# gMedAI-Lab/GAViKO

Hardware: AMD Instinct MI355X
Metric: MRI volumes/sec (fwd+bwd) ViT-B/16 gaviko, 120x160x160 (higher is better)
Workload: dtype bf16

## Files before the change

gaviko_amd/csrc/attention_bwd.hip:

```cpp
#include "attention_common.hpp"
#include "../../include/gaviko_hip.h"

namespace gvk {

template <int QT, bool DROP>
__global__ __launch_bounds__(256, 2) void attn_bwd_dkdv_kernel(const bf16* __restrict__ qkv, const bf16* __restrict__ d_o,
                                                            const float* __restrict__ lse, const float* __restrict__ delta,
                                                            bf16* __restrict__ dqkv, int T, int H, int ld_qkv, int ld_o, float dk_scale,
                                                            AttnDrop dr, int need_rows) {
  constexpr int NSB = QT / 32;
  constexpr int kTileQ = QT * 128;
  constexpr int kBuf = 2 * kTileQ + 2 * 128 * 4;
  extern __shared__ __attribute__((aligned(16))) char smem[];
  int bh, kblk;
  xcd_group_block(blockIdx.x, (T + 127) / 128, gridDim.x / ((T + 127) / 128), bh, kblk);
  const int b = bh / H, head = bh - b * H, k0 = kblk * 128;
  if (k0 >= need_rows) return;
  const int lane = lane_id(), wave = wave_id();
  const int r31 = lane & 31, hh = lane >> 5;
  const int inner = H * 64;
  const bf16* qbase = qkv + (size_t)b * T * ld_qkv + head * 64;
  const bool active = k0 + wave * 32 < T;

  const int key = k0 + wave * 32 + r31;
  const int keyc = min(key, T - 1);
  bf16x8 kf[4], vf[4];
#pragma unroll
  for (int ks = 0; ks < 4; ++ks) {
    kf[ks] = *(const bf16x8*)(qbase + inner + (size_t)keyc * ld_qkv + 16 * ks + 8 * hh);
    vf[ks] = *(const bf16x8*)(qbase + 2 * inner + (size_t)keyc * ld_qkv + 16 * ks + 8 * hh);
  }
  [[maybe_unused]] unsigned int akey = 0u;
  if constexpr (DROP) akey = attn_key(dr.seed + *dr.seed_ptr, b * H + head);

  const int nqt = (T + QT - 1) / QT;
  const int nB = (int)gridDim.x / (((T + 127) / 128) * H);
  const __amdgpu_buffer_rsrc_t rq = __builtin_amdgcn_make_buffer_rsrc((void*)qkv, 0, nB * T * ld_qkv * 2, 0x00020000);
  const __amdgpu_buffer_rsrc_t rd = __builtin_amdgcn_make_buffer_rsrc((void*)d_o, 0, nB * T * ld_o * 2, 0x00020000);
  const __amdgpu_buffer_rsrc_t rl = __builtin_amdgcn_make_buffer_rsrc((void*)(wave < 2 ? lse : delta), 0, nB * H * T * 4, 0x00020000);
  const int rsub = lane >> 3, slot = lane & 7;
  int voq[NSB], vod[NSB];
#pragma unroll
  for (int r = 0; r < NSB; ++r) {
    const int row = r * 32 + wave * 8 + rsub;
    const int col = head * 64 + ((slot ^ attn_swz(row)) << 3);
    voq[r] = ((b * T + row) * ld_qkv + col) * 2;
    vod[r] = ((b * T + row) * ld_o + col) * 2;
  }
  const int lrow = (wave & 1) * 64 + lane;
  const int vol = ((b * H + head) * T + lrow) * 4;
  auto stage = [&](int buf, int qt) {
    char* sQ = smem + buf * kBuf;
    char* sD = sQ + kTileQ;
    char* sL = sD + kTileQ;
    const bool last = qt == nqt - 1;
    const int soq = qt * QT * ld_qkv * 2, sod = qt * QT * ld_o * 2, sol = qt * QT * 4;
#pragma unroll
    for (int r = 0; r < NSB; ++r) {
      const int over = last ? max(qt * QT + r * 32 + wave * 8 + rsub - (T - 1), 0) : 0;
      const int vq = voq[r] - over * ld_qkv * 2, vd = vod[r] - over * ld_o * 2;
      __builtin_amdgcn_raw_ptr_buffer_load_lds(rq, (GVK_LDS void*)(sQ + (r * 32 + wave * 8) * 128), 16, vq, soq, 0, 0);
      __builtin_amdgcn_raw_ptr_buffer_load_lds(rd, (GVK_LDS void*)(sD + (r * 32 + wave * 8) * 128), 16, vd, sod, 0, 0);
    }
    const int overl = last ? max(qt * QT + lrow - (T - 1), 0) : 0;
    const int vl = vol - overl * 4;
    __builtin_amdgcn_raw_ptr_buffer_load_lds(rl, (GVK_LDS void*)(sL + (wave >> 1) * 512 + (wave & 1) * 256), 4, vl, sol, 0, 0);
  };

  f32x16 dkt[2], dvt[2];
#pragma unroll
  for (int i = 0; i < 2; ++i) { dkt[i] = f32x16{}; dvt[i] = f32x16{}; }
  const bf16x8 sel_s = aug_sel_first(true, hh);
  [[maybe_unused]] const bf16x8 sel_d = aug_sel_second(hh);
  const int g = lane >> 4, tq = (lane & 15) >> 2, tp = lane & 3;
  stage(0, 0);
  __syncthreads();
  for (int qt = 0; qt < nqt; ++qt) {
    const int buf = qt & 1;
    if (qt + 1 < nqt) stage(buf ^ 1, qt + 1);
    if (active) {
      const char* sQ0 = smem + buf * kBuf;
      const char* sD0 = sQ0 + kTileQ;
      const float* sL0 = (const float*)(sD0 + kTileQ);
      auto scores = [&](int sub, f32x16& s, f32x16& dp) {
        const int qrow0 = qt * QT + sub * 32;
        const char* sQ = sQ0 + sub * 32 * 128;
        const char* sD = sD0 + sub * 32 * 128;
        const float l2 = sL0[sub * 32 + r31] * 1.44269504088896340736f;
        const float dl = DROP ? 0.f : sL0[128 + sub * 32 + r31];
        const bf16x8 qaug = aug_const(l2, qrow0 + r31 >= T, dl, hh);
        s = __builtin_amdgcn_mfma_f32_32x32x16_bf16(qaug, sel_s, f32x16{}, 0, 0, 0);
        if constexpr (DROP) dp = f32x16{};
        else dp = __builtin_amdgcn_mfma_f32_32x32x16_bf16(qaug, sel_d, f32x16{}, 0, 0, 0);
#pragma unroll
        for (int ks = 0; ks < 4; ++ks) {
          const int chunk = 2 * ks + hh;
          const bf16x8 qa = *(const bf16x8*)(sQ + r31 * 128 + ((chunk ^ attn_swz(r31)) << 4));
          const bf16x8 da = *(const bf16x8*)(sD + r31 * 128 + ((chunk ^ attn_swz(r31)) << 4));
          s = __builtin_amdgcn_mfma_f32_32x32x16_bf16(qa, kf[ks], s, 0, 0, 0);
          dp = __builtin_amdgcn_mfma_f32_32x32x16_bf16(da, vf[ks], dp, 0, 0, 0);
        }
      };
      auto soft = [&](int sub, f32x16& s, f32x16& dp) {
        [[maybe_unused]] const int qrow0 = qt * QT + sub * 32;
#pragma unroll
        for (int r = 0; r < 16; ++r) {
          const float pr = __builtin_amdgcn_exp2f(s[r]);
          if constexpr (DROP) {
            const unsigned int qq = (unsigned int)(qrow0 + (r & 3) + 8 * (r >> 2) + 4 * hh);
            const float mm = attn_drop_scale(akey, qq * (unsigned int)T + (unsigned int)key, dr.thresh, dr.inv_keep);
            const float dlr = sL0[128 + sub * 32 + (r & 3) + 8 * (r >> 2) + 4 * hh];
            s[r] = pr * mm;
            dp[r] = pr * (dp[r] * mm - dlr);
          } else {
            s[r] = pr;
          }
        }
        if constexpr (!DROP) {
#pragma unroll
          for (int r = 0; r < 16; r += 2) {
            typedef float f32x2_ __attribute__((ext_vector_type(2)));
            const f32x2_ pp = {s[r], s[r + 1]}, dd = {dp[r], dp[r + 1]};
            const f32x2_ o = pp * dd;
            dp[r] = o[0]; dp[r + 1] = o[1];
          }
        }
      };
      auto grads = [&](int sub, const f32x16& s, const f32x16& dp) {
        const char* sQ = sQ0 + sub * 32 * 128;
        const char* sD = sD0 + sub * 32 * 128;
#pragma unroll
        for (int sk = 0; sk < 2; ++sk) {
          bf16x8 pf, dsf;
#pragma unroll
          for (int j = 0; j < 8; ++j) { pf[j] = (bf16)s[8 * sk + j]; dsf[j] = (bf16)dp[8 * sk + j]; }
          const int q0r = 16 * sk + 4 * (g >> 1);
#pragma unroll
          for (int db = 0; db < 2; ++db) {
            const int chunk = db * 4 + 2 * (g & 1) + (tp >> 1);
            const int ra = q0r + tq, rb = q0r + 8 + tq;
            const int oa = ra * 128 + ((chunk ^ attn_swz(ra)) << 4) + (tp & 1) * 8;
            const int ob = rb * 128 + ((chunk ^ attn_swz(rb)) << 4) + (tp & 1) * 8;
            const bf16x4 da0 = lds_read_tr16(sD + oa), da1 = lds_read_tr16(sD + ob);
            const bf16x4 qa0 = lds_read_tr16(sQ + oa), qa1 = lds_read_tr16(sQ + ob);
            const bf16x8 dof = {da0[0], da0[1], da0[2], da0[3], da1[0], da1[1], da1[2], da1[3]};
            const bf16x8 qf = {qa0[0], qa0[1], qa0[2], qa0[3], qa1[0], qa1[1], qa1[2], qa1[3]};
            dvt[db] = __builtin_amdgcn_mfma_f32_32x32x16_bf16(dof, pf, dvt[db], 0, 0, 0);
            dkt[db] = __builtin_amdgcn_mfma_f32_32x32x16_bf16(qf, dsf, dkt[db], 0, 0, 0);
          }
        }
      };
      constexpr bool PIPE = !DROP;
      f32x16 sc[PIPE ? 2 : 1], dpc[PIPE ? 2 : 1];
      if constexpr (PIPE) scores(0, sc[0], dpc[0]);
#pragma unroll
      for (int sub = 0; sub < NSB; ++sub) {
        const bool more = sub + 1 < NSB && qt * QT + (sub + 1) * 32 < T;
        constexpr int kCurMask = PIPE ? 1 : 0;
        const int cur = sub & kCurMask;
        if constexpr (PIPE) {
          if (more) scores(sub + 1, sc[(sub + 1) & kCurMask], dpc[(sub + 1) & kCurMask]);
        } else {
          scores(sub, sc[0], dpc[0]);
        }
        if constexpr (PIPE) __builtin_amdgcn_sched_barrier(0);
        soft(sub, sc[cur], dpc[cur]);
        if constexpr (PIPE) __builtin_amdgcn_sched_barrier(0);
        grads(sub, sc[cur], dpc[cur]);
        if constexpr (PIPE) __builtin_amdgcn_sched_barrier(0);
        if (!more) break;
      }
    }
    __syncthreads();
  }
  if (!active) return;
  const int kw = k0 + wave * 32;
  bf16* dk_rows = dqkv + ((size_t)b * T + kw) * ld_qkv + inner + head * 64;
  store_rows_t(dkt, dk_scale, smem + wave * 8192, dk_rows, (size_t)ld_qkv, T - kw, lane);
  store_rows_t(dvt, 1.0f, smem + wave * 8192 + 4096, dk_rows + inner, (size_t)ld_qkv, T - kw, lane);
}

template <int KB, bool DROP>
__global__ __launch_bounds__(256, 2) void attn_bwd_dq_kernel(const bf16* __restrict__ qkv, const bf16* __restrict__ o_fwd, const bf16* __restrict__ d_o,
                                                          const float* __restrict__ lse, float* __restrict__ delta,
                                                          bf16* __restrict__ dqkv, int T, int H, int ld_qkv, int ld_o, float scale,
                                                          AttnDrop dr, int need_rows) {
  constexpr int NKB = KB / 32;
  constexpr int kTileBytes = KB * 128;
  extern __shared__ __attribute__((aligned(16))) char smem[];
  int bh, qblk;
  xcd_group_block(blockIdx.x, (T + 127) / 128, gridDim.x / ((T + 127) / 128), bh, qblk);
  const int b = bh / H, head = bh - b * H, q0 = qblk * 128;
  const int lane = lane_id(), wave = wave_id();
  const int r31 = lane & 31, hh = lane >> 5;
  const int inner = H * 64;
  const bf16* base = qkv + (size_t)b * T * ld_qkv + head * 64;
  const bool active = q0 + wave * 32 < T;
  const int q = q0 + wave * 32 + r31;
  const int qc = min(q, T - 1);
  bf16x8 qf[4], dof[4];
  float del = 0.f;
#pragma unroll
  for (int ks = 0; ks < 4; ++ks) {
    qf[ks] = *(const bf16x8*)(base + (size_t)qc * ld_qkv + 16 * ks + 8 * hh);
    dof[ks] = *(const bf16x8*)(d_o + ((size_t)b * T + qc) * ld_o + head * 64 + 16 * ks + 8 * hh);
    const bf16x8 of = *(const bf16x8*)(o_fwd + ((size_t)b * T + qc) * ld_o + head * 64 + 16 * ks + 8 * hh);
#pragma unroll
    for (int j = 0; j < 8; ++j) del += (float)of[j] * (float)dof[ks][j];
  }
  del = half_sum(del);
  if (hh == 0 && q < T) delta[((size_t)b * H + head) * T + q] = del;
  if (q0 >= need_rows) return;
  [[maybe_unused]] unsigned int akey = 0u, qoff = 0u;
  if constexpr (DROP) {
    akey = attn_key(dr.seed + *dr.seed_ptr, b * H + head);
    qoff = (unsigned int)q * (unsigned int)T;
  }
  const float l2 = lse[((size_t)b * H + head) * T + qc] * 1.44269504088896340736f;
  const bf16x8 qaug = aug_const(l2, true, DROP ? 0.f : del, hh);
  [[maybe_unused]] const bf16x8 sel_d = aug_sel_second(hh);

  const int nkt = (T + KB - 1) / KB;
  const int nB = (int)gridDim.x / (((T + 127) / 128) * H);
  const __amdgpu_buffer_rsrc_t rsrc = __builtin_amdgcn_make_buffer_rsrc((void*)qkv, 0, nB * T * ld_qkv * 2, 0x00020000);
  const int rsub = lane >> 3, slot = lane & 7;
  int vo[NKB], vo_last[NKB];
#pragma unroll
  for (int r = 0; r < NKB; ++r) {
    const int row = r * 32 + wave * 8 + rsub;
    const int col = inner + head * 64 + ((slot ^ attn_swz(row)) << 3);
    vo[r] = ((b * T + row) * ld_qkv + col) * 2;
    vo_last[r] = ((b * T + row - max((nkt - 1) * KB + row - (T - 1), 0)) * ld_qkv + col) * 2;
  }
  auto stage = [&](int buf, int kt) {
    char* sK = smem + buf * 2 * kTileBytes;
    char* sV = sK + kTileBytes;
#pragma unroll
    for (int r = 0; r < NKB; ++r) {
      const int v = (kt == nkt - 1) ? vo_last[r] : vo[r];
      const int so = kt * KB * ld_qkv * 2;
      __builtin_amdgcn_raw_ptr_buffer_load_lds(rsrc, (GVK_LDS void*)(sK + (r * 32 + wave * 8) * 128), 16, v, so, 0, 0);
      __builtin_amdgcn_raw_ptr_buffer_load_lds(rsrc, (GVK_LDS void*)(sV + (r * 32 + wave * 8) * 128), 16, v, so + inner * 2, 0, 0);
    }
  };

  f32x16 dqt[2];
  dqt[0] = f32x16{};
  dqt[1] = f32x16{};
  const int g = lane >> 4, tq = (lane & 15) >> 2, tp = lane & 3;
  stage(0, 0);
  __syncthreads();
  for (int kt = 0; kt < nkt; ++kt) {
    const int buf = kt & 1;
    if (kt + 1 < nkt) stage(buf ^ 1, kt + 1);
    if (active) {
      const char* sK = smem + buf * 2 * kTileBytes;
      const char* sV = sK + kTileBytes;
      auto scores = [&](int kb, f32x16& st, f32x16& dpt) {
        const int row = kb * 32 + r31;
        const bf16x8 sel_s = aug_sel_first(kt * KB + row >= T, hh);
        st = __builtin_amdgcn_mfma_f32_32x32x16_bf16(sel_s, qaug, f32x16{}, 0, 0, 0);
        if constexpr (DROP) dpt = f32x16{};
        else dpt = __builtin_amdgcn_mfma_f32_32x32x16_bf16(sel_d, qaug, f32x16{}, 0, 0, 0);
#pragma unroll
        for (int ks = 0; ks < 4; ++ks) {
          const int chunk = 2 * ks + hh;
          const int off = row * 128 + ((chunk ^ attn_swz(row)) << 4);
          const bf16x8 ka = *(const bf16x8*)(sK + off);
          const bf16x8 va = *(const bf16x8*)(sV + off);
          st = __builtin_amdgcn_mfma_f32_32x32x16_bf16(ka, qf[ks], st, 0, 0, 0);
          dpt = __builtin_amdgcn_mfma_f32_32x32x16_bf16(va, dof[ks], dpt, 0, 0, 0);
        }
      };
      auto soft = [&](int kb, f32x16& st, f32x16& dpt) {
#pragma unroll
        for (int r = 0; r < 16; ++r) {
          float dpv = dpt[r];
          if constexpr (DROP) {
            const int key = kt * KB + kb * 32 + (r & 3) + 8 * (r >> 2) + 4 * hh;
            dpv = dpv * attn_drop_scale(akey, qoff + (unsigned int)key, dr.thresh, dr.inv_keep) - del;
          }
          if constexpr (DROP) st[r] = __builtin_amdgcn_exp2f(st[r]) * dpv;
          else st[r] = __builtin_amdgcn_exp2f(st[r]);
        }
        if constexpr (!DROP) {
#pragma unroll
          for (int r = 0; r < 16; r += 2) {
            typedef float f32x2_ __attribute__((ext_vector_type(2)));
            const f32x2_ pp = {st[r], st[r + 1]}, dd = {dpt[r], dpt[r + 1]};
            const f32x2_ o = pp * dd;
            st[r] = o[0]; st[r + 1] = o[1];
          }
        }
      };
      auto grads = [&](int kb, const f32x16& st) {
#pragma unroll
        for (int s2 = 0; s2 < 2; ++s2) {
          bf16x8 dsf;
#pragma unroll
          for (int j = 0; j < 8; ++j) dsf[j] = (bf16)st[8 * s2 + j];
          const int key0 = kb * 32 + 16 * s2 + 4 * (g >> 1);
#pragma unroll
          for (int db = 0; db < 2; ++db) {
            const int chunk = db * 4 + 2 * (g & 1) + (tp >> 1);
            const int ra = key0 + tq, rb = key0 + 8 + tq;
            const bf16x4 ka0 = lds_read_tr16(sK + ra * 128 + ((chunk ^ attn_swz(ra)) << 4) + (tp & 1) * 8);
            const bf16x4 ka1 = lds_read_tr16(sK + rb * 128 + ((chunk ^ attn_swz(rb)) << 4) + (tp & 1) * 8);
            const bf16x8 kt8 = {ka0[0], ka0[1], ka0[2], ka0[3], ka1[0], ka1[1], ka1[2], ka1[3]};
            dqt[db] = __builtin_amdgcn_mfma_f32_32x32x16_bf16(kt8, dsf, dqt[db], 0, 0, 0);
          }
        }
      };
      f32x16 sc[2], dpc[2];
      scores(0, sc[0], dpc[0]);
#pragma unroll
      for (int kb = 0; kb < NKB; ++kb) {
        if (kb + 1 < NKB) scores(kb + 1, sc[(kb + 1) & 1], dpc[(kb + 1) & 1]);
        __builtin_amdgcn_sched_barrier(0);
        soft(kb, sc[kb & 1], dpc[kb & 1]);
        __builtin_amdgcn_sched_barrier(0);
        grads(kb, sc[kb & 1]);
        __builtin_amdgcn_sched_barrier(0);
      }
    }
    __syncthreads();
  }
  if (!active) return;
  const int qw = q0 + wave * 32;
  store_rows_t(dqt, scale, smem + wave * 4096, dqkv + ((size_t)b * T + qw) * ld_qkv + head * 64, (size_t)ld_qkv, T - qw, lane);
}

__global__ __launch_bounds__(256) void attn_delta_kernel(const bf16* __restrict__ o_fwd, const bf16* __restrict__ d_o, float* __restrict__ delta, int M,
                                                         int T, int H, int ld_o) {
  const int gid = blockIdx.x * 256 + threadIdx.x;
  const int c = gid & 7, rh = gid >> 3;
  const int row = min(rh / H, M - 1), head = rh - (rh / H) * H;
  const size_t off = (size_t)row * ld_o + head * 64 + c * 8;
  const bf16x8 a = *(const bf16x8*)(o_fwd + off), b = *(const bf16x8*)(d_o + off);
  float v = 0.f;
#pragma unroll
  for (int j = 0; j < 8; ++j) v += (float)a[j] * (float)b[j];
  v += __shfl_xor(v, 1, 64);
  v += __shfl_xor(v, 2, 64);
  v += __shfl_xor(v, 4, 64);
  if (c == 0 && rh < M * H) {
    const int bb = row / T, t = row - bb * T;
    delta[((size_t)bb * H + head) * T + t] = v;
  }
}

__device__ __forceinline__ int ds_unit(int keyl, int g, int h) {
  return keyl * 64 + ((g ^ ((keyl >> 2) & 3)) << 4) + ((h ^ ((keyl >> 4) & 1)) << 3);
}

template <int QT, int VAR>
__global__ __launch_bounds__(256, 2) void attn_bwd_fused_kernel(const bf16* __restrict__ qkv, const bf16* __restrict__ d_o, const float* __restrict__ lse,
                                                             const float* __restrict__ delta, bf16* __restrict__ dqkv, float* dq_acc, int* prog,
                                                             int* xcc_tab, int* status, int T, int H, int ld_qkv, int ld_o, float scale, float dk_scale) {
  constexpr int NSB = QT / 32;
  constexpr int kTileQ = QT * 128;
  constexpr int kBuf = 2 * kTileQ + 2 * 128 * 4;
  constexpr int kDS = 128 * 64;
  constexpr int kImg = NSB * kDS;
  static_assert(2 * kImg >= 128 * 128, "the dS^T images first hold the K tile");
  extern __shared__ __attribute__((aligned(16))) char smem[];
  char* const sDSbase = smem + 2 * kBuf;
  int* const stab = (int*)(sDSbase + 2 * kImg);
  const int nkb = (T + 127) / 128, nqt = (T + QT - 1) / QT;
  int bh, kblk;
  xcd_group_block(blockIdx.x, nkb, gridDim.x / nkb, bh, kblk);
  const int b = bh / H, head = bh - b * H, k0 = kblk * 128;
// ... 181 lines not shown
      for (int sb = 0; sb < NSB; ++sb)
#pragma unroll
        for (int qh = 0; qh < 2; ++qh) {
          const int q = qt * QT + sb * 32 + 16 * qh + li;
          const bf16x4 o = {(bf16)(hdq[sb][qh][0] * scale), (bf16)(hdq[sb][qh][1] * scale), (bf16)(hdq[sb][qh][2] * scale), (bf16)(hdq[sb][qh][3] * scale)};
          if (q < T) *(bf16x4*)(dqkv + ((size_t)b * T + q) * ld_qkv + head * 64 + 16 * wave + 4 * G) = o;
        }
    } else if (plain) {
#pragma unroll
      for (int sb = 0; sb < NSB; ++sb)
#pragma unroll
        for (int qh = 0; qh < 2; ++qh) *(f32x4*)((char*)accb + aoff + sb * 8192 + qh * 1024) = hdq[sb][qh];
    } else {
#pragma unroll
      for (int sb = 0; sb < NSB; ++sb)
#pragma unroll
        for (int qh = 0; qh < 2; ++qh)
          __builtin_amdgcn_raw_buffer_store_b128(__builtin_bit_cast(u32x4, hdq[sb][qh]), racc, aoff + sb * 8192 + qh * 1024, 0, 16);
    }
    pend_word = qt;
    pend_val = (last || (VAR & 39) != 0) ? 0 : ppos + 1;
  };

  int qt = start, pos, succ;
  chain(qt, pos, succ);
  if constexpr ((VAR & 1) != 0) pos = 0;
  const int xall = __hip_atomic_load((GVK_GLOBAL int*)(xrow + min(lane, nkb - 1)), __ATOMIC_RELAXED, __HIP_MEMORY_SCOPE_AGENT);
  __builtin_amdgcn_s_waitcnt(0x0F70);
  int xs = succ >= 0 && succ < 64 ? __builtin_amdgcn_readlane(xall, succ & 63) : 0;
  int pv = 0;
  if (nqt > 1) stage(1, start + 1 < nqt ? start + 1 : 0);
  scores(0, 0, start * QT);
  soft();
  int par = 0;
  [[maybe_unused]] unsigned long long ph[6] = {0, 0, 0, 0, 0, 0}, tprev = 0;
#define GVK_PH(k)                                                             \
  if constexpr ((VAR & 64) != 0) {                                            \
    const unsigned long long tnow = __builtin_amdgcn_s_memtime();             \
    if (j >= 2 && j < nqt - 2) ph[k] += tnow - tprev;                         \
    tprev = tnow;                                                             \
  }
  for (int j = 0; j < nqt; ++j) {
    const int buf = j & 1;
    const bool lastm = (VAR & 2) ? true : pos == nkb - 1;
    char* sDS = sDSbase + par * kImg;
    GVK_PH(5)
    grads(buf, 0, sDS);
#pragma unroll
    for (int sb = 1; sb < NSB; ++sb) {
      scores(buf, sb, qt * QT + sb * 32);
      soft();
      grads(buf, sb, sDS + sb * kDS);
    }
    GVK_PH(1)
    if constexpr ((VAR & 128) == 0) asm volatile("s_waitcnt vmcnt(0)" : "+v"(pv) : : "memory");
    GVK_PH(2)
    if constexpr ((VAR & 16) == 0) {
      if (wave == 0 && pos > 0 && pv != pos) {
        for (unsigned spins = 0;; ++spins) {
          __builtin_amdgcn_s_sleep(4);
          pv = __hip_atomic_load((GVK_GLOBAL int*)(progb + qt * 32), __ATOMIC_RELAXED, __HIP_MEMORY_SCOPE_AGENT);
          if (pv == pos) break;
          if (spins > (1u << 16)) { if (lane == 0) atomicAdd(status, 1); break; }
        }
#ifdef GVK_DIAG
        if (lane == 0) atomicAdd(status + 1, 1);
#endif
      }
    }
    if constexpr ((VAR & 128) != 0) {
      __builtin_amdgcn_s_waitcnt(0xC07F);
      __builtin_amdgcn_s_barrier();
    } else {
      __syncthreads();
    }
    GVK_PH(3)
    if (pend_word >= 0 && threadIdx.x == 0)
      __hip_atomic_store((GVK_GLOBAL int*)(progb + pend_word * 32), pend_val, __ATOMIC_RELAXED, __HIP_MEMORY_SCOPE_AGENT);
    pend_word = -1;
    const int h_qt = qt, h_pos = pos;
    const bool h_last = lastm, h_add = pos > 0, h_plain = (VAR & 8) == 0 && xs == my_xcc + 1;
    f32x4 hdq[NSB][2];
    u32x4 hld[NSB][2];
#pragma unroll
    for (int sb = 0; sb < NSB; ++sb)
#pragma unroll
      for (int qh = 0; qh < 2; ++qh) hld[sb][qh] = u32x4{0u, 0u, 0u, 0u};
    if constexpr ((VAR & 37) == 0) {
      const int aoff = qt * NSB * 8192 + wave * 2048 + lane * 16;
#pragma unroll
      for (int sb = 0; sb < NSB; ++sb)
#pragma unroll
        for (int qh = 0; qh < 2; ++qh)
          hld[sb][qh] = __builtin_amdgcn_raw_buffer_load_b128(racc, aoff + sb * 8192 + qh * 1024, 0, 16);
    }
    int qtn = qt + 1 < nqt ? qt + 1 : 0;
    if (j + 1 < nqt) {
      if (j + 2 < nqt) stage(buf, qtn + 1 < nqt ? qtn + 1 : 0);
      chain(qtn, pos, succ);
      if constexpr ((VAR & 1) != 0) pos = 0;
      xs = succ >= 0 && succ < 64 ? __builtin_amdgcn_readlane(xall, succ & 63) : 0;
    } else {
      qtn = qt;
    }
    const int bufn = j + 1 < nqt ? buf ^ 1 : buf;
    if constexpr ((VAR & 16) == 0) {
      if (wave == 0) asm volatile("global_load_dword %0, %1, %2 sc1" : "=v"(pv) : "v"(0), "s"(progb + qtn * 32) : "memory");
    }
    GVK_PH(4)
#pragma unroll
    for (int sb = 0; sb < NSB; ++sb) {
      hdq[sb][0] = f32x4{0.f, 0.f, 0.f, 0.f};
      hdq[sb][1] = f32x4{0.f, 0.f, 0.f, 0.f};
      if constexpr ((VAR & 4) == 0) {
#pragma unroll
        for (int kk = 0; kk < 4; ++kk)
#pragma unroll
          for (int qh = 0; qh < 2; ++qh) {
            const char* im = sDS + sb * kDS + kk * 2048;
            const bf16x4 b0 = lds_read_tr16(im + dsr[qh][0]), b1 = lds_read_tr16(im + dsr[qh][1]);
            const bf16x8 bb = {b0[0], b0[1], b0[2], b0[3], b1[0], b1[1], b1[2], b1[3]};
            hdq[sb][qh] = __builtin_amdgcn_mfma_f32_16x16x32_bf16(ktf[kk], bb, hdq[sb][qh], 0, 0, 0);
          }
      }
    }
    scores(bufn, 0, qtn * QT);
    GVK_PH(0)
    if constexpr ((VAR & 4) == 0 && (VAR & 32) == 0) finish(hdq, hld, h_qt, h_pos, h_add, h_last, h_plain);
    if constexpr ((VAR & 32) != 0) {
      if (hdq[0][0][0] + hdq[NSB - 1][1][3] == 123.456f) atomicAdd(status + 3, 1);
    }
    soft();
    qt = qtn;
    par ^= 1;
  }
#undef GVK_PH
  if constexpr ((VAR & 64) != 0) {
    if (lane == 0 && (blockIdx.x == 3 || blockIdx.x == 100 || blockIdx.x == 259))
      for (int k = 0; k < 6; ++k) ((unsigned long long*)(status + 16))[(blockIdx.x == 3 ? 0 : blockIdx.x == 100 ? 1 : 2) * 32 + wave * 8 + k] = ph[k];
  }
  asm volatile("s_waitcnt vmcnt(0)" ::: "memory");
  __syncthreads();
  if (threadIdx.x == 0) {
    if (pend_word >= 0) __hip_atomic_store((GVK_GLOBAL int*)(progb + pend_word * 32), pend_val, __ATOMIC_RELAXED, __HIP_MEMORY_SCOPE_AGENT);
    __hip_atomic_store((GVK_GLOBAL int*)(xrow + kblk), 0, __ATOMIC_RELAXED, __HIP_MEMORY_SCOPE_AGENT);
  }
  if (!active) return;
  const int kw = k0 + wave * 32;
  bf16* dk_rows = dqkv + ((size_t)b * T + kw) * ld_qkv + inner + head * 64;
  store_rows_t(dkt, dk_scale, smem + wave * 8192, dk_rows, (size_t)ld_qkv, T - kw, lane);
  store_rows_t(dvt, 1.0f, smem + wave * 8192 + 4096, dk_rows + inner, (size_t)ld_qkv, T - kw, lane);
}

template <int KB, bool DROP>
static int launch_attn_bwd(const void* qkv, const void* out, const void* dout, const float* lse, float* delta, void* dqkv, int B, int T, int H,
                           int ld_qkv, int ld_out, float scale, AttnDrop dr, hipStream_t s, int need_rows = 1 << 30) {
  const float dk_scale = 0.69314718055994530942f;
  const dim3 grid(((T + 127) / 128) * H * B);
  constexpr unsigned lds_kv = 2 * (2 * KB * 128 + 2 * 128 * 4), lds_q = 2 * 2 * KB * 128;
  static bool attr = false;
  if (!attr) {
    hipError_t e = hipFuncSetAttribute(reinterpret_cast<const void*>(&attn_bwd_dq_kernel<KB, DROP>), hipFuncAttributeMaxDynamicSharedMemorySize, lds_q);
    if (e == hipSuccess) e = hipFuncSetAttribute(reinterpret_cast<const void*>(&attn_bwd_dkdv_kernel<KB, DROP>), hipFuncAttributeMaxDynamicSharedMemorySize, lds_kv);
    if (e != hipSuccess) return set_error(-3, "hipFuncSetAttribute(attn_bwd): %s", hipGetErrorString(e));
    attr = true;
  }
  GVK_LAUNCH((attn_bwd_dq_kernel<KB, DROP>), grid, dim3(256), lds_q, s, (const bf16*)qkv, (const bf16*)out, (const bf16*)dout, lse, delta, (bf16*)dqkv, T, H,
             ld_qkv, ld_out, scale, dr, need_rows);
  int rc = check_launch("attention_bwd/dq");
  if (rc) return rc;
  GVK_LAUNCH((attn_bwd_dkdv_kernel<KB, DROP>), grid, dim3(256), lds_kv, s, (const bf16*)qkv, (const bf16*)dout, lse, (const float*)delta, (bf16*)dqkv, T, H,
             ld_qkv, ld_out, dk_scale, dr, need_rows);
  return check_launch("attention_bwd/dkdv");
}

}

extern "C" int gvk_attention_bwd_bf16_dropout(const void* qkv, const void* out, const void* dout, const float* lse, float* delta, void* dqkv, int B,
                                              int T, int H, int ld_qkv, int ld_out, float scale, float drop_p, uint64_t seed, const void* seed_ptr,
                                              void* stream) {
  using namespace gvk;
  GVK_REQUIRE(qkv && out && dout && lse && delta && dqkv, "gvk_attention_bwd_bf16: null pointer");
  GVK_REQUIRE(B > 0 && T > 0 && H > 0, "gvk_attention_bwd_bf16: empty shape");
  GVK_REQUIRE(ld_qkv >= 3 * H * 64 && ld_qkv % 8 == 0 && ld_out >= H * 64 && ld_out % 8 == 0,
              "gvk_attention_bwd_bf16: head dim is fixed at 64; ld_qkv=%d ld_out=%d inconsistent with H=%d", ld_qkv, ld_out, H);
  GVK_REQUIRE(drop_p >= 0.f && drop_p < 1.f && (drop_p == 0.f || seed_ptr != nullptr), "gvk_attention_bwd_bf16: drop_p in [0,1) and a seed word");
  GVK_REQUIRE(drop_p == 0.f || (int64_t)T * T < (int64_t)1 << 32, "gvk_attention_bwd_bf16: the dropout mask index (query*T + key) is 32-bit");
  GVK_REQUIRE((int64_t)B * T * ld_qkv * 2 < (int64_t)1 << 31, "gvk_attention_bwd_bf16: the qkv tensor must stay below 2 GiB (32-bit buffer offsets)");
  const AttnDrop dr{seed, (const unsigned long long*)seed_ptr, drop_threshold_u32(drop_p), drop_p > 0.f ? 1.f / (1.f - drop_p) : 1.f};
  hipStream_t s = (hipStream_t)stream;
  int kb = ((T + 95) / 96 * 96 < (T + 127) / 128 * 128) ? 96 : 128;
  if (getenv("GAVIKO_HIP_ATTN_KB") && (atoi(getenv("GAVIKO_HIP_ATTN_KB")) == 96 || atoi(getenv("GAVIKO_HIP_ATTN_KB")) == 128)) kb = atoi(getenv("GAVIKO_HIP_ATTN_KB"));
  if (drop_p > 0.f)
    return launch_attn_bwd<96, true>(qkv, out, dout, lse, delta, dqkv, B, T, H, ld_qkv, ld_out, scale, dr, s);
  return kb == 96 ? launch_attn_bwd<96, false>(qkv, out, dout, lse, delta, dqkv, B, T, H, ld_qkv, ld_out, scale, dr, s)
                  : launch_attn_bwd<128, false>(qkv, out, dout, lse, delta, dqkv, B, T, H, ld_qkv, ld_out, scale, dr, s);
}

static constexpr int kFusedQT = 64;
static size_t fused_slabs(int B, int T, int H) { return (size_t)B * H * ((T + kFusedQT - 1) / kFusedQT) * (kFusedQT / 32); }
static size_t fused_ws_cap(size_t ws_bytes) { return ws_bytes < 1024 ? 0 : (ws_bytes - 1024) / (8192 + 128 + 4); }
static size_t fused_status_off(size_t ws_bytes) { return (fused_ws_cap(ws_bytes) * 132 + 255) / 256 * 256; }

extern "C" size_t gvk_attention_bwd_ws_bytes(int B, int T, int H) {
  if (B <= 0 || T <= 0 || H <= 0) return 0;
  return fused_slabs(B, T, H) * (8192 + 128 + 4) + 1024;
}
extern "C" size_t gvk_attention_bwd_status_offset(size_t ws_bytes) { return fused_status_off(ws_bytes); }

extern "C" int gvk_attention_bwd_bf16_fused(const void* qkv, const void* out, const void* dout, const float* lse, float* delta, void* dqkv, void* ws,
                                            size_t ws_bytes, int B, int T, int H, int ld_qkv, int ld_out, float scale, void* stream) {
  using namespace gvk;
  GVK_REQUIRE(qkv && out && dout && lse && delta && dqkv && ws, "gvk_attention_bwd_bf16_fused: null pointer");
  GVK_REQUIRE(B > 0 && T > 0 && H > 0, "gvk_attention_bwd_bf16_fused: empty shape");
  GVK_REQUIRE(ld_qkv >= 3 * H * 64 && ld_qkv % 8 == 0 && ld_out >= H * 64 && ld_out % 8 == 0,
              "gvk_attention_bwd_bf16_fused: head dim is fixed at 64; ld_qkv=%d ld_out=%d inconsistent with H=%d", ld_qkv, ld_out, H);
  GVK_REQUIRE((int64_t)B * T * ld_qkv * 2 < (int64_t)1 << 31, "gvk_attention_bwd_bf16_fused: the qkv tensor must stay below 2 GiB (32-bit buffer offsets)");
  const size_t need = gvk_attention_bwd_ws_bytes(B, T, H);
  GVK_REQUIRE(ws_bytes >= need && ((uintptr_t)ws & 255) == 0, "gvk_attention_bwd_bf16_fused: workspace of %zu bytes (256-byte aligned) needed, %zu given", need, ws_bytes);
  GVK_REQUIRE(fused_ws_cap(ws_bytes) >= fused_slabs(B, T, H), "gvk_attention_bwd_bf16_fused: workspace layout cannot hold %zu slabs", fused_slabs(B, T, H));
  const size_t off_status = fused_status_off(ws_bytes), off_acc = off_status + 256;
  const size_t nsub = (size_t)((T + kFusedQT - 1) / kFusedQT) * (kFusedQT / 32);
  GVK_REQUIRE(nsub * 8192 < ((size_t)1 << 31) && (T + 127) / 128 <= 256, "gvk_attention_bwd_bf16_fused: sequence too long (32-bit slab offsets, 256 key blocks)");
  hipStream_t s = (hipStream_t)stream;
  constexpr unsigned lds = 2 * (2 * kFusedQT * 128 + 2 * 128 * 4) + 2 * (kFusedQT / 32) * 128 * 64 + 1024;
  static bool attr = false;
  if (!attr) {
    hipError_t e = hipFuncSetAttribute(reinterpret_cast<const void*>(&attn_bwd_fused_kernel<kFusedQT, 0>), hipFuncAttributeMaxDynamicSharedMemorySize, lds);
#ifdef GVK_DIAG
    auto set1 = [&](const void* f) { if (e == hipSuccess) e = hipFuncSetAttribute(f, hipFuncAttributeMaxDynamicSharedMemorySize, lds); };
    set1(reinterpret_cast<const void*>(&attn_bwd_fused_kernel<kFusedQT, 1>)); set1(reinterpret_cast<const void*>(&attn_bwd_fused_kernel<kFusedQT, 3>));
    set1(reinterpret_cast<const void*>(&attn_bwd_fused_kernel<kFusedQT, 7>)); set1(reinterpret_cast<const void*>(&attn_bwd_fused_kernel<kFusedQT, 8>));
    set1(reinterpret_cast<const void*>(&attn_bwd_fused_kernel<kFusedQT, 11>)); set1(reinterpret_cast<const void*>(&attn_bwd_fused_kernel<kFusedQT, 15>));
    set1(reinterpret_cast<const void*>(&attn_bwd_fused_kernel<kFusedQT, 16>)); set1(reinterpret_cast<const void*>(&attn_bwd_fused_kernel<kFusedQT, 64>)); set1(reinterpret_cast<const void*>(&attn_bwd_fused_kernel<kFusedQT, 33>)); set1(reinterpret_cast<const void*>(&attn_bwd_fused_kernel<kFusedQT, 129>)); set1(reinterpret_cast<const void*>(&attn_bwd_fused_kernel<kFusedQT, 144>));
#endif
    if (e != hipSuccess) return set_error(-3, "hipFuncSetAttribute(attn_bwd_fused): %s", hipGetErrorString(e));
    attr = true;
  }
  const int M = B * T;
  GVK_LAUNCH(attn_delta_kernel, dim3((unsigned)(((size_t)M * H * 8 + 255) / 256)), dim3(256), 0, s, (const bf16*)out, (const bf16*)dout, delta, M, T, H, ld_out);
  int rc = check_launch("attention_bwd/delta");
  if (rc) return rc;
  const float dk_scale = 0.69314718055994530942f;
  char* w = (char*)ws;
  const dim3 grid(((T + 127) / 128) * H * B);
#define GVK_FUSED(V)                                                                                                                          \
  GVK_LAUNCH((attn_bwd_fused_kernel<kFusedQT, V>), grid, dim3(256), lds, s, (const bf16*)qkv, (const bf16*)dout, lse, (const float*)delta, \
             (bf16*)dqkv, (float*)(w + off_acc), (int*)w, (int*)w + fused_ws_cap(ws_bytes) * 32, (int*)(w + off_status), T, H, ld_qkv, ld_out, scale, dk_scale)
#ifdef GVK_DIAG
  const int var = diag_env("GAVIKO_HIP_ATTN_VAR") ? atoi(diag_env("GAVIKO_HIP_ATTN_VAR")) : 0;
  if (var == 1) GVK_FUSED(1); else if (var == 3) GVK_FUSED(3); else if (var == 7) GVK_FUSED(7); else if (var == 8) GVK_FUSED(8);
  else if (var == 11) GVK_FUSED(11); else if (var == 15) GVK_FUSED(15); else if (var == 16) GVK_FUSED(16); else if (var == 64) GVK_FUSED(64); else if (var == 33) GVK_FUSED(33); else if (var == 129) GVK_FUSED(129); else if (var == 144) GVK_FUSED(144); else
#endif
  GVK_FUSED(0);
#undef GVK_FUSED
  return check_launch("attention_bwd/fused");
}

extern "C" int gvk_attention_bwd_bf16_rows(const void* qkv, const void* out, const void* dout, const float* lse, float* delta, void* dqkv, int B,
                                           int T, int H, int ld_qkv, int ld_out, float scale, int need_rows, void* stream) {
  using namespace gvk;
  GVK_REQUIRE(qkv && out && dout && lse && delta && dqkv, "gvk_attention_bwd_bf16_rows: null pointer");
  GVK_REQUIRE(B > 0 && T > 0 && H > 0 && need_rows > 0, "gvk_attention_bwd_bf16_rows: empty shape");
  GVK_REQUIRE(ld_qkv >= 3 * H * 64 && ld_qkv % 8 == 0 && ld_out >= H * 64 && ld_out % 8 == 0,
              "gvk_attention_bwd_bf16_rows: head dim is fixed at 64; ld_qkv=%d ld_out=%d inconsistent with H=%d", ld_qkv, ld_out, H);
  GVK_REQUIRE((int64_t)B * T * ld_qkv * 2 < (int64_t)1 << 31, "gvk_attention_bwd_bf16_rows: the qkv tensor must stay below 2 GiB (32-bit buffer offsets)");
  const AttnDrop dr{0, nullptr, 0u, 1.f};
  const int kb = ((T + 95) / 96 * 96 < (T + 127) / 128 * 128) ? 96 : 128;
  return kb == 96 ? launch_attn_bwd<96, false>(qkv, out, dout, lse, delta, dqkv, B, T, H, ld_qkv, ld_out, scale, dr, (hipStream_t)stream, need_rows)
                  : launch_attn_bwd<128, false>(qkv, out, dout, lse, delta, dqkv, B, T, H, ld_qkv, ld_out, scale, dr, (hipStream_t)stream, need_rows);
}

extern "C" int gvk_attention_bwd_bf16(const void* qkv, const void* out, const void* dout, const float* lse, float* delta, void* dqkv, int B,
                                      int T, int H, int ld_qkv, int ld_out, float scale, void* stream) {
  return gvk_attention_bwd_bf16_dropout(qkv, out, dout, lse, delta, dqkv, B, T, H, ld_qkv, ld_out, scale, 0.f, 0, nullptr, stream);
}
```

gaviko_amd/engine.py:

```python
from __future__ import annotations

import os
from typing import Dict, List, Optional

import torch

from . import lib as L
from . import ops
from .engine_common import (GRAPH_WARMUP, PLAN_TIMING, SEED_EMB, SEED_LAYER, SEED_PROMPT, USE_GRAPHS, _ABLATE, _EPI_NAMES, _SIDE_STREAMS, Names,
                            _on)
from .engine_common import evp_highpass_operator
from .engine_gaviko import GavikoPaths
from .engine_peft import PeftPaths

GEMM_MARKS = None


_BB_KINDS = ("vit", "adaptformer", "gaviko", "dvpt", "evp", "vpt", "ssf")


class Engine(GavikoPaths, PeftPaths):
    def __init__(self, kind: str, cfg: dict, params: Dict[str, torch.nn.Parameter], depth, heads, dim, mlp_dim):
        self.kind, self.cfg, self.p = kind, cfg, params
        self.depth, self.heads, self.C, self.mlp = depth, heads, dim, mlp_dim
# ... 161 lines not shown
        if stale:
            conv = self._d(names[0]).reshape(self.C, self.Kp).contiguous()
            w["conv"] = ops.to_operand(conv, None if self.fp32 else w.get("conv"), self.adt)
        if not stale and (not need_dgrad or self._have_dgrad):
            return
        for i in range(self.depth):
            for tag, nm in (("qkv", self.names.qkv_weight(i)), ("out", self.names.attn(i) + ".to_out.0.weight"),
                            ("fc1", self.names.mlp(i) + ".net.1.weight"), ("fc2", self.names.mlp(i) + ".net.4.weight")):
                src = self._d(nm).contiguous()
                if stale and tag == "fc2" and self._fuse_up:
                    buf = w.get(f"fc2{i}")
                    if buf is None:
                        buf = w[f"fc2{i}"] = torch.zeros((self.C, self.ldx), dtype=self.adt, device=src.device)
                    buf[:, :self.mlp].copy_(src)
                elif stale:
                    w[f"{tag}{i}"] = ops.to_operand(src, None if self.fp32 else w.get(f"{tag}{i}"), self.adt)
                if need_dgrad and (stale or not self._have_dgrad):
                    w[f"{tag}{i}_t"] = ops.transpose_operand(src, w.get(f"{tag}{i}_t"), self.adt)
        self._have_dgrad = self._have_dgrad and not stale or need_dgrad
        self._w16_version = version

    def _fold_deps(self) -> List[str]:
        n = []
        for i in range(1, self.depth):
            a = self.names.attn(i)
            n += [self.names.qkv_weight(i), a + ".norm.weight", a + ".norm.bias"]
        return n

    def _ensure_fold(self) -> bool:
        if not self._fold_ln1:
            return False
        names = self._fold_deps()
        version = tuple(self.p[n]._version for n in names) + tuple(self.p[n].data_ptr() for n in names)
        if version == self._fold_version and self._fold:
            return True
        for i in range(1, self.depth):
            a = self.names.attn(i)
            Wq, g, b = self._d(self.names.qkv_weight(i)), self._d(a + ".norm.weight"), self._d(a + ".norm.bias")
            w16 = ops.to_operand((Wq * g[None, :]).contiguous(), self._fold.get(f"w{i}"), self.adt)
            self._fold[f"w{i}"] = w16
            for key, val in ((f"c1_{i}", w16.float().sum(1)),
                             (f"c2_{i}", (Wq * b[None, :]).sum(1))):
                if key in self._fold:
                    self._fold[key].copy_(val)
                else:
                    self._fold[key] = val.contiguous()
        self._fold_version = version
        return True

    def _seed_base(self, train: bool) -> int:
        rank = 0
        try:
            import torch.distributed as dist
            if dist.is_available() and dist.is_initialized():
                rank = dist.get_rank()
        except Exception:
            rank = 0
        x = (torch.initial_seed() & 0xFFFFFFFFFFFF) * 0x9E3779B97F4A7C15 + (rank + 1) * 0xBF58476D1CE4E5B9 + (0x94D049BB133111EB if train else 0)
        x &= (1 << 64) - 1
        x ^= x >> 31
        return 0x5EED0000 ^ (x & 0x3FFFFFFFFFFF0000)

    def invalidate_weights(self, names=None) -> None:
        if names is None or any(n in self._shadowed for n in names):
            self._w16_version = None
        if names is None or any(n in self._fold_names for n in names):
            self._fold_version = None

    def workspace(self, B: int, device, train: bool, keep_attn: bool = False, tag: Optional[str] = None):
        key = (B, train, str(device)) + (("attn",) if keep_attn else ()) + ((tag,) if tag else ())
        if key in self._wss:
            self._ws = self._wss[key]
            return self._ws
        C, T, N, M = self.C, self.T, self.N, B * self.T
        z = lambda r, c, dt: ops.act_zeros(r, c, dt, device)
        f32, bf16 = torch.float32, self.adt
        nsave = self.depth if (train or keep_attn) else 1
        ws = {"key": key, "B": B, "M": M}
        ws["img"] = torch.zeros((B, 1) + tuple(g * p for g, p in zip(self.grid, self.patch)), device=device)
        ws["logits"] = torch.zeros((B, self.K), device=device)
        ws["dlogits"] = torch.zeros((B, self.K), device=device)
        ws["seed"] = torch.full((1,), self._seed_base(train), dtype=torch.int64, device=device)
        ws["cols"] = z(B * N, self.Kp, bf16)
        ws["G"] = [z(M, C, f32) for _ in range(self.depth + 1)] if train else [z(M, C, f32), z(M, C, f32)]
        ws["G1"] = [z(M, C, f32) for _ in range(nsave)]
        ws["xn"] = z(M, C, bf16)
        ws["qkv"] = [z(M, 3 * C, bf16) for _ in range(nsave)]
        ws["ctx"] = [z(M, C, bf16) for _ in range(nsave)]
        ws["lse"] = [torch.zeros((B, self.heads, T), device=device) for _ in range(nsave)]
        ws["pre"] = [z(M, self.ldx, bf16) for _ in range(nsave)] if train else [None]
        ws["act"] = z(M, self.ldx, bf16)
        if self._fuse_up:
            ws["act"][:, self.mlp + 3 * self.Lat: self.mlp + 3 * self.Lat + 2] = 1.0
        ws["stat"] = [[torch.zeros(M, device=device) for _ in range(4)] for _ in range(nsave)]
        ws["pooled"] = torch.zeros((B, C), device=device)
        if self._fold_ln1:
            ws["xg16"] = z(M, C, bf16)
            ws["spart"] = torch.zeros((C // 64) * M * 2, device=device)
        if self.kind == "gaviko":
            Lt, P, BN = self.Lat, self.P, B * N
            ws["Lc"] = [torch.zeros((BN, C), device=device) for _ in range((self.depth + 1) if train else 2)]
            mk = lambda *s: torch.zeros(s, device=device)
            ws["mw"] = [dict(mean=mk(BN), rstd=mk(BN), lat=mk(BN, Lt), qkv=mk(BN, 3 * Lt), ctx=mk(BN, Lt), lse=mk(BN)) for _ in range(nsave)]
            ws["gp"] = [dict(zx=mk(M, Lt), xl=mk(M, Lt), zl=mk(BN, Lt), ll=mk(BN, Lt), imp=mk(B, P), gw=mk(B), enh=mk(B, P, Lt),
                             prm=mk(B, P, Lt), qg=mk(B, P, Lt), ql=mk(B, P, Lt), cg=mk(B, P, Lt), cl=mk(B, P, Lt), lse_g=mk(B, P),
                             lse_l=mk(B, P)) for _ in range(nsave)]
        if self.kind == "evp":
            mk = lambda *s_: torch.zeros(s_, device=device)
            BN, Lp = B * N, self.Lp
            ws["xc"] = z(BN, C, f32)
            ws["hp"] = torch.zeros_like(ws["img"])
            ws["hcols"] = z(BN, self.Kp, f32)
            ws["hc"] = z(BN, 64, f32)
            ws["ev"] = dict(e=mk(BN, Lp), s=mk(BN, Lp), pre=[mk(BN, Lp) for _ in range(nsave)], u=[mk(BN, Lp) for _ in range(nsave)],
                            tmp=z(BN, C, f32))
            if train:
                ws["evb"] = dict(du=mk(BN, Lp), dpre=mk(BN, Lp), ds_tmp=mk(BN, Lp), ds=mk(BN, Lp))
                ws["scratch"] = mk(max(ops.outer_scratch_elems(Lp, self.Kp), 128 * C))
                ws["rscratch"] = mk(32 * (Lp * Lp + Lp + 64))
        if self.kind == "dvpt":
            mk = lambda *s_: torch.zeros(s_, device=device)
            ws["dv"] = [dict(z=mk(M, self.Lat), enh=mk(B, self.P, self.Lat), lse=mk(B, self.P)) for _ in range(nsave)]
        if self.kind == "adaptformer":
            ws["xa"] = z(M, C, bf16)
            ws["ad"] = [dict(mean=torch.zeros(M, device=device), rstd=torch.zeros(M, device=device), h16=z(M, self.adim, bf16))
                        for _ in range(nsave)]
            if train:
                ws["dh16"] = z(M, self.adim, bf16)
                ws["h32"] = torch.zeros((M, self.adim), device=device)
                ws["dh32"] = torch.zeros((M, self.adim), device=device)
        if self.kind == "melo":
            ws["merge32"] = torch.zeros((3 * C, C), device=device)
            if train:
                mk = lambda *s_: torch.zeros(s_, device=device)
                ws["dq32"], ws["dv32"] = mk(M, C), mk(M, C)
                ws["lu"] = dict(uq=mk(M, self.r), uv=mk(M, self.r), duq=mk(M, self.r), duv=mk(M, self.r))
        if self.kind == "vpt":
            R = (self.depth if self.deep else 1) * self.P
            ws["vproj"] = torch.zeros((R, C), device=device)
            ws["Go"] = z(M, C, f32)
            if train:
                ws["dvproj"] = torch.zeros((R, C), device=device)
                ws["dGv"] = z(M, C, f32)
        if train:
            ws["dG"] = [z(M, C, f32), z(M, C, f32)]
            ws["dG16"] = z(M, C, bf16)
            ws["dpre"] = z(M, self.mlp, bf16)
            ws["dx32"] = z(M, C, f32)
            if self._dy16:
                ws["dx16b"] = z(M, C, bf16)
            ws["dctx"] = z(M, C, bf16)
            ws["dqkv"] = z(M, 3 * C, bf16)
            ws["delta"] = torch.zeros((B, self.heads, T), device=device)
            if self.kind == "gaviko":
                Lt, P, BN = self.Lat, self.P, B * N
                mk = lambda *s: torch.zeros(s, device=device)
                ng = ops.gpa_gate_param_count(Lt, P)
                ws["dL"] = [mk(BN, C), mk(BN, C)]
                ws["dGb"] = ops.act_zeros(M, C, torch.float32, device)
                ws["bw"] = dict(dcomb=mk(M, Lt), dimp=mk(B, P), dgw_part=mk(B, P), dqg=mk(B, P, Lt), dql=mk(B, P, Lt), dcg=mk(B, P, Lt),
                                dcl=mk(B, P, Lt), delta_g=mk(B, P), delta_l=mk(B, P), dprm=mk(B, P, Lt), dcls=mk(B, Lt),
                                gate_partials=mk(B, ng), dzx=mk(M, Lt), dzl=[mk(BN, Lt), mk(BN, Lt)],
                                dctx=mk(BN, Lt), dqkv=mk(BN, 3 * Lt), wdelta=mk(BN), dlat=mk(BN, Lt), Q=mk(Lt, C), S=mk(Lt))
                ws["scratch"] = mk(max(ops.outer_scratch_elems(Lt, C), 128 * C, 64 * 3 * Lt * Lt, 64 * ng))
                ws["rscratch"] = mk(32 * (ng + 2 * Lt * Lt + 3 * Lt + 3 * Lt * Lt + 64))
                ws["scratch_l"] = mk(max(ops.outer_scratch_elems(Lt, C), 128 * C))
                ws["rscratch_l"] = mk(32 * (3 * Lt * Lt + Lt + 64))
                if self._pgrad:
                    nct = (C + 63) // 64
                    ws["pscratch"] = mk(ops.param_grads_scratch_elems(Lt, [nct, nct], [ng, Lt * Lt, Lt, Lt * Lt, Lt, Lt]))
                    ws["pscratch_l"] = mk(ops.param_grads_scratch_elems(Lt, [nct, nct, (3 * Lt + 63) // 64], []))
                    ws["ptick"] = torch.zeros(ops.PGRAD_TICKETS, dtype=torch.int32, device=device)
                    ws["ptick_l"] = torch.zeros(ops.PGRAD_TICKETS, dtype=torch.int32, device=device)
            elif self.kind == "dvpt":
                Lt, P = self.Lat, self.P
                mk = lambda *s_: torch.zeros(s_, device=device)
                ws["dvb"] = dict(dcomb=mk(M, Lt), dz=mk(M, Lt), delta=mk(B, P))
                ws["scratch"] = mk(max(ops.outer_scratch_elems(Lt, C), 128 * C))
                ws["rscratch"] = mk(32 * (Lt + 64))
            elif self.kind == "evp":
                pass
            else:
                if self.kind == "ssf":
                    ws["ssf_scratch"] = torch.zeros(64 * 2 * max(self.mlp, 3 * C), device=device)
                    ws["ssf_tmp"] = torch.zeros(2 * C, device=device)
                    ws["ssf_stat"] = [torch.zeros(M, device=device), torch.zeros(M, device=device)]
                lat = {"adaptformer": 64, "melo": getattr(self, "r", 4)}.get(self.kind, 1)
                ws["scratch"] = torch.zeros(max(128 * C, ops.outer_scratch_elems(lat, C)), device=device)
        self._ws = self._wss[key] = ws
        return ws

    def _stream(self, name):
        st = self._streams.get(name)
        if st is None:
            key = (torch.cuda.current_device(), name)
            st = _SIDE_STREAMS.get(key)
            if st is not None:
                self._streams[name] = st
                return st
            st = self._streams[name] = _SIDE_STREAMS[key] = torch.cuda.Stream()
            if "sidenop" in _ABLATE or f"{name}nop" in _ABLATE:
                L.load().gvk_plan_nop_stream(st.cuda_stream)
        return st

    def _ev_record(self, stream):
        if "noevents" in _ABLATE:
            return None
        if self._recording:
            rc = L.load().gvk_plan_event_record(stream.cuda_stream)
            if rc < 0:
                L.check(rc, "gvk_plan_event_record")
            return rc
        ev = torch.cuda.Event()
        ev.record(stream)
        return ev

    def _bucket_mark(self, kind, layer):
        if not self._want_bucket_marks:
            return
        cur = torch.cuda.current_stream()
        if self._recording:
            rc = L.load().gvk_plan_event_record_fenced(cur.cuda_stream)
            if rc < 0:
                L.check(rc, "gvk_plan_event_record_fenced")
            self._bucket_marks[(kind, layer)] = rc
        else:
            ev = torch.cuda.Event()
            ev.record(cur)
            self._bucket_marks[(kind, layer)] = ev

    def _mark(self, name):
        if self._recording and PLAN_TIMING:
            self._marks.append((name, self._ev_record(torch.cuda.current_stream())))

    def _ev_wait(self, stream, ev):
        if "noevents" in _ABLATE or ("nowait" in _ABLATE and stream.cuda_stream == torch.cuda.current_stream().cuda_stream):
            return
        if self._recording:
            L.check(L.load().gvk_plan_event_wait(stream.cuda_stream, ev), "gvk_plan_event_wait")
        else:
            stream.wait_event(ev)

    def _wait(self, waiter, on):
        cur = torch.cuda.current_stream()
        src = cur if on is None else self._stream(on)
        dst = cur if waiter is None else self._stream(waiter)
        self._ev_wait(dst, self._ev_record(src))

    def _run(self, tag, key, fn):
        k = (tag,) + key + (torch.cuda.current_stream().cuda_stream,)
        g = self._graphs.get(k)
        self._last_run = ("eager", None)
        if g is not None:
            L.check(L.load().gvk_plan_replay(g), "gvk_plan_replay")
            self._last_run = ("replayed", g)
            return
        n = self._calls.get(k, 0)
        self._calls[k] = n + 1
        if not USE_GRAPHS or n < GRAPH_WARMUP:
            fn()
            return
        lib = L.load()
        L.check(lib.gvk_plan_begin(), "gvk_plan_begin")
        self._recording = True
        self._marks, self._gemm_marks = [], []
        self._bucket_marks = {}
        try:
            if GEMM_MARKS is not None:
                cur = torch.cuda.current_stream()
                self._gemm_marks.append(("__empty__", 0.0, None, None, self._ev_record(cur), self._ev_record(cur)))
            fn()
        except BaseException:
            lib.gvk_plan_abort()
            raise
        finally:
            self._recording = False
        pid = lib.gvk_plan_end()
        if pid < 0:
            L.check(pid, "gvk_plan_end")
        self._graphs[k] = pid
        self.plan_marks[pid] = (tag, self._marks)
        self.plan_bucket_marks[pid] = dict(self._bucket_marks)
        self._last_run = ("recorded", pid)
        if self._gemm_marks:
            self.plan_gemm_marks[pid] = self._gemm_marks
        return

    def forward(self, img: torch.Tensor, train: bool, drop: Optional[dict] = None, keep_attn: bool = False, ws_tag: Optional[str] = None) -> torch.Tensor:
        L.require_device()
        if not img.is_cuda:
            raise L.GavikoHipError("input volume must be on the HIP device: gaviko_amd has no CPU path")
        if img.dim() != 5 or img.shape[1] != 1 or tuple(img.shape[2:]) != tuple(g * p for g, p in zip(self.grid, self.patch)):
            raise L.GavikoHipError(f"expected img [B,1,{self.grid[0] * self.patch[0]},{self.grid[1] * self.patch[1]},"
                                   f"{self.grid[2] * self.patch[2]}], got {tuple(img.shape)}")
        B = img.shape[0]
        drop = drop or {}
        sv = {"B": B, "train": train, "keep": train or keep_attn, "attn_drop": float(drop.get("attn_drop", 0.0)), "proj_drop": float(drop.get("proj_drop", 0.0))}
        sv["bdrop"], sv["edrop"], sv["pdrop"] = (float(drop.get(k, 0.0)) for k in ("dropout", "emb_dropout", "prompt_dropout"))
        if (sv["bdrop"] > 0 or sv["edrop"] > 0 or sv["pdrop"] > 0) and self.kind not in ("vit", "melo", "vpt", "adaptformer", "gaviko", "dvpt", "evp", "ssf"):
            raise L.GavikoHipError(f"backbone dropout > 0 in training mode: unknown kind {self.kind!r}")
        self.refresh_weights(need_dgrad=train)
        ws = self.workspace(B, img.device, train, keep_attn=keep_attn and not train, tag=ws_tag)
        if img.data_ptr() != ws["img"].data_ptr():
            ws["img"].copy_(img.detach())
        bb = frozenset()
        if train and self.kind in _BB_KINDS:
# ... 435 lines not shown
            self._mark("b:begin")
            self._backward_head(ws, sv, gv, True)
        dGout, dGin = ws["dG"][0], ws["dG"][1]
        if gaviko and ((self.depth - 1 - hi) & 1):
            dGout = ws["dGb"]
        vpt_deep = self.kind == "vpt" and self.deep
        if vpt_deep and ((self.depth - 1 - hi) & 1):
            dGout = ws["dGv"]
        if gaviko:
            loc, gpa = self._stream("loc"), self._stream("gpa")
            self._wait("gpa", None)
            self._wait("loc", None)
        bb = sv.get("bb") or ()
        dy16 = bool(self._dy16 and not bb and not sv["wgrad"])
        frozen = gaviko and not bb and sv.get("bdrop", 0.0) <= 0 and not sv["wgrad"]
        top = self._panels(B, sum(self._pool_rows())) if (frozen and first) else {}
        bot = self._panels(B, self.P) if (frozen and last and self.P > 0 and not self._igrad) else {}
        prev_scl = None
        for i in range(hi, lo - 1, -1):
            M = B * self.Ts[i]
            T = self.Ts[i]
            par = (self.depth - 1 - i) & 1
            if gaviko:
                with torch.cuda.stream(gpa):
                    self._gpa_bwd_core(ws, sv, gv, i, dGout, M, B, par, project=not self._fuse_proj or i == self.depth - 1)
                    dz_ready = self._ev_record(gpa)
                    self._gpa_bwd_params(ws, sv, gv, i, dGout, M, B, par)
                    self._bucket_mark("gpa", i)
            self._mark(f"b{i}:start")
            self._mlp_block_bwd(ws, sv, gv, i, dGout, dGin, dy16, top if i == self.depth - 1 else {})
            self._mark(f"b{i}:ln2")
            if gaviko:
                self._ev_wait(torch.cuda.current_stream(), dz_ready)
                self._gpa_bwd_scatter_g(ws, i, dGin, M)
                self._mark(f"b{i}:scatter")
                self._mwsa_chain_bwd(ws, sv, gv, i, par, B, loc, dz_ready)
            if gaviko:
                dGout = ws["dGb"] if dGout is ws["dG"][0] else ws["dG"][0]
            self._attn_block_bwd(ws, sv, gv, i, dGin, dGout, dy16, bot if i == 0 else {})
            if gaviko:
                if prev_scl is not None:
                    self._ev_wait(gpa, prev_scl)
                prev_scl = self._scl_done
                self._wait("gpa", None)
            if self.kind == "evp":
                self._evp_bwd_layer(ws, gv, i, dGout, B)
            if self.kind == "ssf" and bb:
                self._ssf_unfold(gv, bb, self._ssf_sites()[1 + 6 * i: 7 + 6 * i])
            self._mark(f"b{i}:end")
            if not gaviko:
                self._bucket_mark("main", i)
            if self.kind == "vpt" and (i == 0 or self.deep):
                if sv.get("pdrop", 0.0) > 0:
                    ops.dropout_rows(dGout, sv["pdrop"], SEED_PROMPT + i, ws["seed"], out32=dGout, M=B * self.P, N=C, rows_in=self.P, rows_out=T, row_off=1)
                ops.rows_batch_sum(dGout, ws["dvproj"][i * self.P: (i + 1) * self.P], None, B, T, 1, self.P, C)
            if vpt_deep and i > 0:
                other = ws["dGv"] if dGout is ws["dG"][0] else ws["dG"][0]
                ops.vpt_repack_bwd(dGout, other, B, self.Ts[i - 1], T, self.P, self.pd, C)
                dGout = other
                ops.to_operand(dGout, ws["dG16"], self.adt)
        if gaviko:
            if last:
                self._mwsa_flush(ws, B, loc, dead=self.prune_dead_rows and lo == 0 and not sv.get("bb") and not self._igrad)
            self._wait(None, "gpa")
            self._wait(None, "loc")
        if last and sv.get("bb"):
            if sv.get("edrop", 0.0) > 0:
                ops.dropout_rows(dGout, sv["edrop"], SEED_EMB, ws["seed"], out32=dGout, M=B * self.T, N=C)
            dlocal = ws["dL"][(self.depth - 1 - lo + 1) & 1] if gaviko else None
            if gaviko and sv.get("edrop", 0.0) > 0:
                ops.dropout_rows(dlocal, sv["edrop"], SEED_EMB + 1, ws["seed"], out32=dlocal, M=B * self.N, N=C)
            if self.kind == "evp":
                dlocal = ws["ev"]["tmp"]
                ops.skinny_up(lat=ws["evb"]["ds"], w=self._evp_state(dGout.device)["We"], out=dlocal, M=B * self.N, C=C, L=self.Lp, w_layout=1,
                              accumulate=0)
            self._bb_embed_grads(ws, gv, sv["bb"], dGout, B, dlocal=dlocal, dlocal_to_pos=gaviko)
        if last and self.kind == "evp":
            self._evp_bwd_finish(ws, gv, B)
        if last and self.kind == "ssf":
            pos = self.p["pos_embedding"].detach()[0]
            ops.ssf_colgrad(dGout, ws["G"][0], self.p["ssf_scale_1"].detach(), self.p["ssf_shift_1"].detach(), gv["ssf_scale_1"], gv["ssf_shift_1"],
                            ws["ssf_scratch"], B * self.N, C, pos=pos[1:], rows_in=self.N, rows_out=T, row_off=1,
                            y_mul=1.0 - sv.get("edrop", 0.0))
            self._ssf_unfold(gv, sv.get("bb") or (), self._ssf_sites()[:1])
        if last and self.kind == "vpt":
            emb_name = "deep_prompt_embeddings" if self.deep else "prompt_embeddings"
            emb = d(emb_name).reshape(-1, self.pd)
            ops.small_linear_bwd(emb, d("prompt_proj.weight"), ws["dvproj"], gv["prompt_proj.weight"], gv["prompt_proj.bias"],
                                 gv[emb_name].view(-1, self.pd), emb.shape[0], self.pd, C)
        if last and (gaviko or self.kind == "dvpt"):
            ops.rows_batch_sum(dGout, gv["prompt_embeddings"].view(self.P, C), gv["prompt_positional_embedding"].view(self.P, C), B, T, 0,
                               self.P, C)
        if last and self._igrad:
            self._input_grad_tail(ws, sv, dGout, B, lo)
        if last:
            self._bucket_mark("main", -1)
        self._mark("b:tail")

    def _mlp_block_bwd(self, ws, sv, gv, i, dGout, dGin, dy16, top):
        w, d, C = self._w16, self._d, self.C
        B, T = sv["B"], self.Ts[i]
        M, m, st = B * T, self.names.mlp(i), ws["stat"][i]
        bb, pd_ = sv.get("bb") or (), sv.get("bdrop", 0.0)
        dvpt, ssf = self.kind == "dvpt", self.kind == "ssf"
        dy_ff = dGout
        if pd_ > 0:
            dy_ff = self._masked_grad(ws, dGout, pd_, SEED_LAYER + 8 * i + 3, bool(bb) or ssf, M)
        if bb:
            self._bb_linear_grads(ws, gv, bb, m + ".net.4", dy_ff, ws["dG16"], ws["sav"]["act"][i] if sv["wgrad"] else None, M, C, self.mlp,
                                  ldx=self.ldx if self.ldx != self.mlp else None)
        if dvpt:
            self._dvpt_bwd_latents(ws, gv, i, dGout, M, B)
        if ssf:
            self._ssf_linear_grad(ws, gv, m, 2, dy_ff, ws["G"][i + 1], M, C, y1=ws["G1"][i], y_mul=1.0 - pd_)
        self._gemm(ws["dG16"], w[f"fc2{i}_t"], M, ws["dpre"], epilogue=ops.EPI_GELU_BWD_BF16, aux=ws["pre"][i], ldaux=self.ldx,
                   drop_p=pd_, seed=SEED_LAYER + 8 * i + 2, seed_ptr=ws["seed"], aux_is_grad=int(sv.get("pre_is_grad", False)), **top)
        if ssf:
            self._ssf_linear_grad(ws, gv, m, 1, ws["dpre"], ws["pre"][i], M, self.mlp)
        if bb:
            self._bb_linear_grads(ws, gv, bb, m + ".net.1", ws["dpre"], ws["dpre"], ws["sav"]["xn2"][i] if sv["wgrad"] else None, M, self.mlp, C)
        self._gemm(ws["dpre"], w[f"fc1{i}_t"], M, ws["dx16b"] if dy16 else ws["dx32"], epilogue=ops.EPI_STORE_BF16 if dy16 else ops.EPI_STORE_F32,
                   **top)
        self._mark(f"b{i}:fc1d")
        if bb:
            self._bb_ln_grads(ws, gv, bb, m + ".net.0", ws["dx32"], ws["G1"][i], st[2], st[3], M)
        if ssf:
            self._ssf_ln_grad(ws, gv, m, ".net.0", ws["dx32"], ws["G1"][i], st[2], st[3], M)
        if top:
            ops.memset_zero(dGin)
        self._ln_bwd(ws, dy16, ws["G1"][i], st[2], st[3], d(m + ".net.0.weight"), M, dx=dGin, dres=dGout,
                     dx16=None if self.kind in ("gaviko", "adaptformer", "dvpt") else ws["dG16"],
                     rows=(B, sum(self._pool_rows()), T) if top else None)
        if dvpt:
            self._dvpt_bwd_scatter(ws, i, dGin, M)
        if self.kind == "adaptformer":
            self._adapter_bwd(ws, gv, i, dGout, dGin, M, refresh_operand=pd_ > 0)

    def _attn_block_bwd(self, ws, sv, gv, i, dGin, dx, dy16, bot):
        w, d, C = self._w16, self._d, self.C
        B, T = sv["B"], self.Ts[i]
        M, a, st = B * T, self.names.attn(i), ws["stat"][i]
        bb, pd_ = sv.get("bb") or (), sv.get("bdrop", 0.0)
        ssf = self.kind == "ssf"
        dy_at = dGin
        if pd_ > 0:
            dy_at = self._masked_grad(ws, dGin, pd_, SEED_LAYER + 8 * i + 1, bool(bb) or ssf, M)
        if ssf:
            self._ssf_linear_grad(ws, gv, a, 2, dy_at, ws["G1"][i], M, C, y1=ws["G"][i], y_mul=1.0 - pd_)
        if bb:
            self._bb_linear_grads(ws, gv, bb, a + ".to_out.0", dy_at, ws["dG16"], ws["ctx"][i], M, C, C)
        self._gemm(ws["dG16"], w[f"out{i}_t"], M, ws["dctx"], epilogue=ops.EPI_STORE_BF16)
        self._mark(f"b{i}:outd")
        ops.attention_bwd(ws["qkv"][i], ws["ctx"][i], ws["dctx"], ws["lse"][i], ws["delta"], ws["dqkv"], B, T, self.heads, 64 ** -0.5,
                          drop_p=pd_, seed=SEED_LAYER + 8 * i, seed_ptr=ws["seed"], q_prescaled=True, need_rows=self.P if bot else None)
        self._mark(f"b{i}:attnb")
        if self.kind == "melo" and i in self.lora_layers:
            self._melo_bwd(ws, gv, i, M)
        if ssf:
            uq = {} if self.fp32 else dict(y0_cols=self.heads * 64, y0_mul=1.0 / self.q_scale)
            self._ssf_linear_grad(ws, gv, a, 1, ws["dqkv"], ws["qkv"][i], M, 3 * C, **uq)
        if bb:
            self._bb_linear_grads(ws, gv, bb, a + ".to_qkv", None, ws["dqkv"], ws["sav"]["xn1"][i] if sv["wgrad"] else None, M, 3 * C, C)
        self._gemm(ws["dqkv"], w[f"qkv{i}_t"], M, ws["dx16b"] if dy16 else ws["dx32"], epilogue=ops.EPI_STORE_BF16 if dy16 else ops.EPI_STORE_F32,
                   **bot)
        if bb:
            self._bb_ln_grads(ws, gv, bb, a + ".norm", ws["dx32"], ws["G"][i], st[0], st[1], M)
        if ssf:
            self._ssf_ln_grad(ws, gv, a, ".norm", ws["dx32"], ws["G"][i], st[0], st[1], M)
        self._mark(f"b{i}:qkvd")
        proj = None
        if self._fuse_proj and i > 0:
            pre_lo, _ = self._gpa_names(i - 1)
            proj = dict(w=d(pre_lo + ".proj_up.weight"), y=ws["bw"]["dcomb"], w_layout=1, L_=self.Lat)
        self._ln_bwd(ws, dy16, ws["G"][i], st[0], st[1], d(a + ".norm.weight"), M, dx=dx, dres=dGin, dx16=None if bot else ws["dG16"],
                     rows=(B, self.P, T) if bot else None, proj=proj)

    def _ln_bwd(self, ws, dy16, x, mean, rstd, gamma, M, *, dx, dres, dx16=None, rows=None, proj=None):
        if dy16:
            ops.layernorm_bwd_dy16(ws["dx16b"], x, mean, rstd, gamma, M, self.C, dx=dx, dres=dres, dx16=dx16, rows=rows, proj=proj)
        elif rows is not None:
            ops.layernorm_bwd_rows(ws["dx32"], x, mean, rstd, gamma, *rows, self.C, dx=dx, dres=dres, dx16=dx16)
        elif proj is not None:
            ops.layernorm_bwd_proj(ws["dx32"], x, mean, rstd, gamma, M, self.C, dx=dx, dres=dres, dx16=dx16, **proj)
        else:
            ops.layernorm_bwd(ws["dx32"], x, mean, rstd, gamma, M, self.C, dx=dx, dres=dres, dx16=dx16)

    def _ig_names(self) -> List[str]:
        head = self.names.head()
        return [n for n, p in self.p.items() if p.requires_grad or n.startswith(head) or self._own_grad_kernels(n)]

    def _ig_scratch_views(self, device, real) -> Dict[str, torch.Tensor]:
        names = [n for n in self._ig_names() if n not in real]
        if not real:
            from .distributed import flat_order
            names = flat_order(tuple(names), self.cfg.get("share_factor", 1) if self.kind == "gaviko" else 1, self.bucket_layers)
        sig = (tuple((n, tuple(self.p[n].shape)) for n in names), str(device))
        sc = self._ig_scratch.get(self._igrad)
        if sc is None or sc["sig"] != sig:
            if sc is not None:
                self._graphs.clear()
                self._calls.clear()
            buf = torch.zeros(max(1, sum(self.p[n].numel() for n in names)), device=device)
            views, off = {}, 0
            for n in names:
                k = self.p[n].numel()
                views[n] = buf[off: off + k].view(self.p[n].shape)
                off += k
            sc = self._ig_scratch[self._igrad] = {"sig": sig, "buf": buf, "views": views}
        return sc["views"]

    def _ig_buffers(self, ws, B, device) -> None:
        C, BN, Kp = self.C, B * self.N, self.Kp
        if "ig" not in ws:
            ig = ws["ig"] = dict(dxc=ops.act_zeros(BN, C, torch.float32, device), dcols=ops.act_zeros(BN, Kp, torch.float32, device))
            if not self.fp32:
                ig["dxc16"] = ops.act_zeros(BN, C, self.adt, device)
            if self.kind == "evp":
                ig["dhc"] = ops.act_zeros(BN, 64, torch.float32, device)
                ig["dhcols"] = ops.act_zeros(BN, Kp, torch.float32, device)
                ig["dhp"] = torch.zeros_like(ws["img"])
                ig["dhp2"] = torch.zeros_like(ws["img"])
            ws["dimg"] = torch.zeros_like(ws["img"])
        w = self._w16
        if "conv_t" not in w:
            w["conv_t"] = torch.zeros((Kp, C), dtype=self.adt, device=device)
        if self.kind == "evp":
            st = self._evp_state(device)
            if "hpT" not in st:
                st["hpT"] = st["hp"].t().contiguous()
                st["WpT"] = torch.zeros((Kp, 64), device=device)
        if self.kind == "ssf":
            return
        cw = self.p[self.names.conv() + ".weight"]
        version = (cw._version, cw.data_ptr())
        if version != self._conv_t_version:
            ops.transpose_operand(self._d(self.names.conv() + ".weight").reshape(C, Kp).contiguous(), w["conv_t"], self.adt)
            self._conv_t_version = version

    def _input_grad_tail(self, ws, sv, dG0, B, lo):
        C, T, N, Kp, BN = self.C, self.T, self.N, self.Kp, B * self.N
        ig, w = ws["ig"], self._w16
        edrop = sv.get("edrop", 0.0)
        premasked = bool(sv.get("bb"))
        src = dG0
        if edrop > 0 and not premasked:
            ops.dropout_rows(dG0, edrop, SEED_EMB, ws["seed"], out32=ws["dx32"], M=B * T, N=C)
            src = ws["dx32"]
        ops.rows_gather(src, ig["dxc"], B, T, N, C, self.row_off)
        if self.kind == "gaviko":
            dlocal = ws["dL"][(self.depth - lo) & 1]
            if edrop > 0 and not premasked:
                ops.dropout_rows(dlocal, edrop, SEED_EMB + 1, ws["seed"], out32=dlocal, M=BN, N=C)
            ops.add2d(ig["dxc"], C, dlocal, C, ig["dxc"], C, BN, C)
        if self.kind == "evp":
            ops.skinny_up(lat=ws["evb"]["ds"], w=self._evp_state(dG0.device)["We"], out=ig["dxc"], M=BN, C=C, L=self.Lp, w_layout=1, accumulate=1)
        if self.kind == "ssf":
            ops.ssf_fold_weight(self.p[self.names.conv() + ".weight"].detach().reshape(C, Kp), self.p["ssf_scale_1"].detach(), w["conv"], w["conv_t"])
        a = ig["dxc"] if self.fp32 else ops.to_operand(ig["dxc"], ig["dxc16"], self.adt)
        ops.gemm_nt(a, w["conv_t"], BN, ig["dcols"], epilogue=ops.EPI_STORE_F32)
        if self.kind == "evp":
            st = self._evp_state(dG0.device)
            ops.pad2d(ws["evb"]["ds"], BN, self.Lp, ig["dhc"], BN, 64)
            ops.transpose_any(st["Wp"], st["WpT"], 64, Kp)
            ops.gemm_nt(ig["dhc"], st["WpT"], BN, ig["dhcols"], epilogue=ops.EPI_STORE_F32)
            ops.unpatchify(ig["dhcols"], ig["dhp"], self.patch)
            ops.evp_highpass_sign(ws["img"], st["hp"], st["dmask"], ig["dhp"], ig["dhp2"])
            ops.evp_highpass_linear(ig["dhp2"], st["hpT"], st["dmask"], ig["dhp"])
            ops.patchify(ig["dhp"], ig["dhcols"], self.patch)
            ops.add2d(ig["dcols"], Kp, ig["dhcols"], Kp, ig["dcols"], Kp, BN, Kp)
        ops.unpatchify(ig["dcols"], ws["dimg"], self.patch)

    def _grad_supported(self, name: str) -> bool:
        return name.startswith(self.names.head()) or self.kind in _BB_KINDS or self._own_grad_kernels(name)

    def _own_grad_kernels(self, name: str) -> bool:
        if self.kind == "vit":
            return False
        if self.kind == "gaviko":
            return ("local_attns" in name or "prompt_projs" in name or name in ("prompt_embeddings", "prompt_positional_embedding"))
        if self.kind == "vpt":
            return name in ("prompt_proj.weight", "prompt_proj.bias", "deep_prompt_embeddings", "prompt_embeddings")
        if self.kind == "adaptformer":
            return "adapter" in name
        if self.kind == "melo":
            return ".linear_a_" in name or ".linear_b_" in name
        if self.kind == "ssf":
            return "ssf_scale_" in name or "ssf_shift_" in name
        if self.kind == "dvpt":
            return "prompt" in name
        if self.kind == "evp":
            return "prompt_generator" in name
        return False

    def _needs_backbone_backward(self) -> bool:
        return any(not n.startswith(self.names.head()) for n in self.trainable_names())
```

gaviko_amd/lib.py:

```python
from __future__ import annotations

import ctypes as C
import os

import torch

_HERE = os.path.dirname(os.path.abspath(__file__))
if os.environ.get("GPU_MAX_HW_QUEUES") is None:
    os.environ["GPU_MAX_HW_QUEUES"] = "8"
    try:
        import sys as _sys
        _t = _sys.modules.get("torch")
        if _t is not None and _t.cuda.is_initialized():
            import warnings as _w
            _w.warn("gaviko_amd: HIP was initialised before gaviko_amd was imported, so GPU_MAX_HW_QUEUES=8 cannot take effect; the three "
                    "streams of a step may share hardware queues (slower, not wrong).  Import gaviko_amd first or export the variable.")
    except Exception:
        pass

ABI_VERSION = 12
DIAG = os.environ.get("GAVIKO_HIP_DIAG", "0") == "1"
LIB_PATH = os.environ.get("GAVIKO_HIP_LIB") or os.path.join(_HERE, "libgaviko_hip_diag.so" if DIAG else "libgaviko_hip.so")


def diag_env(name: str, default=None):
    return os.environ.get(name, default) if DIAG else default


class GemmDesc(C.Structure):
    _fields_ = [
        ("a", C.c_void_p), ("w", C.c_void_p), ("out0", C.c_void_p), ("out1", C.c_void_p),
        ("bias", C.c_void_p), ("res", C.c_void_p), ("aux", C.c_void_p), ("pos", C.c_void_p), ("seed_ptr", C.c_void_p),
        ("M", C.c_int32), ("N", C.c_int32), ("K", C.c_int32),
        ("lda", C.c_int32), ("ldw", C.c_int32), ("ldo", C.c_int32), ("ldres", C.c_int32), ("ldaux", C.c_int32),
        ("epilogue", C.c_int32), ("rows_in", C.c_int32), ("rows_out", C.c_int32), ("row_off", C.c_int32),
        ("tile", C.c_int32), ("drop_p", C.c_float), ("seed", C.c_uint64),
        ("scale_cols", C.c_int32), ("col_scale", C.c_float),
        ("ln_mean", C.c_void_p), ("ln_rstd", C.c_void_p), ("ln_c1", C.c_void_p), ("stat_part", C.c_void_p), ("stat_pivot", C.c_void_p),
        ("m_panels", C.c_int32), ("m_stride", C.c_int32), ("splitk_ws", C.c_void_p), ("splitk_ws_bytes", C.c_uint64),
        ("ksplit", C.c_int32), ("aux_is_grad", C.c_int32),
    ]


def _struct(name, ptrs, ints, floats=(), u64=(), i64=()):
    fields = [(f, C.c_void_p) for f in ptrs] + [(f, C.c_int32) for f in ints] + [(f, C.c_float) for f in floats] + \
             [(f, C.c_uint64) for f in u64] + [(f, C.c_int64) for f in i64]
    return type(name, (C.Structure,), {"_fields_": fields})


SkinnyDownDesc = _struct("SkinnyDownDesc",
                         ["x", "w", "bias", "ln_gamma", "ln_beta", "mean", "rstd", "z", "y", "w2", "y2", "seed_ptr"],
                         ["M", "C", "L", "L2", "act", "w_layout", "act_in"], ["eps", "drop_p"], ["seed"])
SkinnyUpDesc = _struct("SkinnyUpDesc", ["lat", "w", "bias", "res", "out", "lat_override", "seed_ptr", "ln_x", "ln_mean", "ln_rstd", "ln_gamma", "out_bf16",
                                        "alpha_ptr", "gg_x", "w2", "bias2", "z2", "y2", "lat_b", "w_b",
                                        "nx_w", "nx_bias", "nx_ln_gamma", "nx_ln_beta", "nx_mean", "nx_rstd", "nx_lat", "nx_w2", "nx_y2"],
                       ["M", "C", "L", "T", "P", "w_layout", "accumulate", "L2", "act2", "w2_layout", "nx_L2"], ["drop_p", "drop2_p", "nx_eps"],
                       ["seed", "seed2"])
OuterDesc = _struct("OuterDesc", ["narrow", "wide", "lat_override", "mean", "rstd", "ln_gamma", "ln_beta", "scratch", "out", "colsum", "seed_ptr",
                                  "narrow2", "wide2"],
                    ["M", "C", "L", "T", "P", "transposed", "accumulate", "wide_act", "M2"], ["drop_p"], ["seed"])
WindowAttnDesc = _struct("WindowAttnDesc", ["qkv", "ctx", "lse", "dctx", "delta", "dqkv", "seed_ptr"],
                         ["B", "D", "H", "W", "kd", "kh", "kw", "L"], ["scale", "drop_p"], ["seed"])
GpaDesc = _struct("GpaDesc",
                  ["xl", "ll", "ca0_g", "ca0_b", "ca1_w", "ca1_b", "ca3_w", "ca3_b", "gl0_g", "gl0_b", "gl1_w", "gl1_b",
                   "wgq", "bgq", "wlq", "blq", "imp", "gw", "enh", "prm", "qg", "ql", "cg", "cl", "lse_g", "lse_l",
                   "dcomb", "zx", "zl", "dimp", "dgw_part", "dqg", "dql", "dcg", "dcl", "delta_g", "delta_l", "dprm",
                   "dcls", "gate_partials", "dzx", "dzl", "enh16"],
                  ["B", "T", "N", "P", "L", "ld16", "col16"], ["scale"])
SsfColgradDesc = _struct("SsfColgradDesc", ["dy", "y0", "y1", "pos", "s", "t", "ds", "dt", "scratch"],
                         ["M", "N", "ld_dy", "ld_y", "dy_f32", "y0_f32", "rows_in", "rows_out", "row_off", "y0_cols"], ["y0_mul", "y_mul"])
DvptDesc = _struct("DvptDesc", ["z", "enh", "lse", "dcomb", "gate", "bu", "colsum_dy", "delta", "dz", "dgate"], ["B", "T", "P", "L", "C"], ["scale"])
AdamDesc = _struct("AdamDesc", ["ptr_tab", "blk_tab", "grad", "m", "v", "norm_sq"], ["nblocks"],
                   ["lr", "beta1", "beta2", "eps", "bias_c1", "bias_c2", "max_norm"])
LossDesc = _struct("LossDesc", ["logits", "target", "weights", "loss", "dlogits", "meter"], ["B", "K", "kind", "reduction"], ["gamma", "eps"], i64=["ignore_index"])
DropoutDesc = _struct("DropoutDesc", ["x", "out32", "out16", "seed_ptr"], ["M", "N", "ld", "rows_in", "rows_out", "row_off"], ["drop_p"], ["seed"])
RowProjDesc = _struct("RowProjDesc", ["w", "bias", "y", "z", "y_split"], ["L", "w_layout", "act", "ld_split", "col_split"])
LnBwdDy16Desc = _struct("LnBwdDy16Desc", ["dy_bf16", "x", "mean", "rstd", "gamma", "dres", "dx", "dx_bf16", "proj"],
                        ["M", "C", "groups", "rows_per_group", "group_stride"])
ReduceJob = _struct("ReduceJob", ["a", "b", "out", "a2"], ["M", "J", "L", "accumulate", "M2"])
PgradOuter = _struct("PgradOuter", ["narrow", "wide", "narrow2", "wide2", "lat_override", "mean", "rstd", "out", "colsum",
                                    "aff_w", "aff_gamma", "aff_beta", "aff_dgamma", "aff_dbeta", "aff_dbias"],
                     ["M", "M2", "T", "P", "transposed", "accumulate", "C"], ["drop_p"], ["seed"])
HeadDesc = _struct("HeadDesc", ["g", "ln_gamma", "ln_beta", "wh", "bh", "logits", "pooled", "dlogits", "dg", "dwh", "dbh"],
                   ["B", "T", "C", "K", "r0", "R", "accumulate"])

(EPI_STORE_BF16, EPI_BIAS_RES_F32, EPI_BIAS_GELU_BF16, EPI_PATCH_F32, EPI_GELU_BWD_BF16, EPI_STORE_F32, EPI_BIAS_RES_F32_BF16,
 EPI_BIAS_RELU_BF16, EPI_RELU_BWD_BF16) = range(9)

_P, _I, _F, _L = C.c_void_p, C.c_int, C.c_float, C.c_int64
SIGNATURES = {
    "gvk_gemm_nt_bf16": [C.POINTER(GemmDesc), _P],
    "gvk_gemm_nt_f32": [C.POINTER(GemmDesc), _P],
    "gvk_attention_fwd_f32": [_P, _P, _P, _I, _I, _I, _I, _I, _F, _P],
    "gvk_attention_bwd_f32": [_P, _P, _P, _P, _P, _P, _I, _I, _I, _I, _I, _F, _P],
    "gvk_patchify_f32": [_P, _P, _I, _I, _I, _I, _I, _I, _I, _P],
    "gvk_transpose_f32": [_P, _P, _I, _I, _P],
    "gvk_transpose_bf16": [_P, _P, _I, _I, _P],
    "gvk_copy_async": [_P, _P, C.c_size_t, _P],
    "gvk_copy_f32_strided": [_P, _P, _I, _I, _I, _P],
    "gvk_cast_f32_bf16": [_P, _P, _L, _P],
    "gvk_transpose_cast_f32_bf16": [_P, _P, _I, _I, _P],
    "gvk_pack_split_bf16": [_P, _I, _P, _P, _I, _I, _I, _I, _P],
    "gvk_prompt_up_fix": [_P, _P, _P, _P, _I, _I, _I, _I, _I, _P],
    "gvk_layernorm_fwd_fix": [_P, _P, _P, _P, _P, _P, _I, _I, _F, _P, _P, _P, _I, _I, _I, _P],
    "gvk_patchify_bf16": [_P, _P, _I, _I, _I, _I, _I, _I, _I, _P],
    "gvk_layernorm_fwd": [_P, _P, _P, _P, _P, _P, _P, _I, _I, _F, _P],
    "gvk_layernorm_bwd": [_P, _P, _P, _P, _P, _P, _P, _P, _I, _I, _P],
    "gvk_layernorm_bwd_rows": [_P, _P, _P, _P, _P, _P, _P, _P, _I, _I, _I, _I, _P],
    "gvk_layernorm_bwd_affine": [_P, _P, _P, _P, _P, _P, _P, _I, _I, _I, _P],
    "gvk_attention_fwd_bf16": [_P, _P, _P, _I, _I, _I, _I, _I, _F, _P],
    "gvk_qkv_prescale_bf16": [_P, _I, _I, _I, _F, _P],
    "gvk_prompt_up_fix_stats": [_P, _P, _P, _P, _P, _P, _I, _P, _P, _P, _I, _I, _I, _I, _I, _F, _P],
    "gvk_attention_bwd_bf16": [_P, _P, _P, _P, _P, _P, _I, _I, _I, _I, _I, _F, _P],
    "gvk_attention_bwd_bf16_rows": [_P, _P, _P, _P, _P, _P, _I, _I, _I, _I, _I, _F, _I, _P],
    "gvk_attention_bwd_bf16_fused": [_P, _P, _P, _P, _P, _P, _P, C.c_size_t, _I, _I, _I, _I, _I, _F, _P],
    "gvk_attention_colsum_bf16": [_P, _P, _P, _I, _P, _I, _I, _I, _I, _I, _I, _P],
    "gvk_rollout_step": [_P, _P, _P, _I, _I, _I, _P],
    "gvk_unpatchify_f32": [_P, _P, _P, _P, _I, _I, _I, _I, _I, _I, _I, _I, _F, _F, _P],
    "gvk_patch_reduce_f32": [_P, _P, _I, _I, _I, _I, _I, _I, _I, _I, _P],
    "gvk_evp_highpass_sign": [_P, _P, _P, _P, _P, _I, _I, _I, _I, _P],
    "gvk_evp_highpass_linear": [_P, _P, _P, _P, _I, _I, _I, _I, _I, _P],
    "gvk_attention_fwd_f32_dropout": [_P, _P, _P, _I, _I, _I, _I, _I, _F, _F, C.c_uint64, _P, _P],
    "gvk_attention_bwd_f32_dropout": [_P, _P, _P, _P, _P, _P, _I, _I, _I, _I, _I, _F, _F, C.c_uint64, _P, _P],
    "gvk_attention_fwd_bf16_dropout": [_P, _P, _P, _I, _I, _I, _I, _I, _F, _F, C.c_uint64, _P, _P],
    "gvk_attention_bwd_bf16_dropout": [_P, _P, _P, _P, _P, _P, _I, _I, _I, _I, _I, _F, _F, C.c_uint64, _P, _P],
    "gvk_skinny_down": [C.POINTER(SkinnyDownDesc), _P],
    "gvk_skinny_up": [C.POINTER(SkinnyUpDesc), _P],
    "gvk_outer_reduce": [C.POINTER(OuterDesc), _P],
    "gvk_small_wgrad": [_P, _P, _P, _P, _I, _I, _I, _I, _P],
    "gvk_ln_lowrank_affine": [_P, _P, _P, _P, _P, _P, _P, _P, _P, _I, _I, _I, _P],
    "gvk_colsum": [_P, _P, _P, _I, _I, _I, _P],
    "gvk_reduce_batch": [C.POINTER(ReduceJob), _I, _P, _P],
    "gvk_param_grads": [C.POINTER(PgradOuter), _I, C.POINTER(ReduceJob), _I, _P, _L, _P, _I, _P, _I, _I, _P],
    "gvk_window_attn_fwd": [C.POINTER(WindowAttnDesc), _P],
    "gvk_window_attn_bwd": [C.POINTER(WindowAttnDesc), _P],
    "gvk_gpa_fwd": [C.POINTER(GpaDesc), _P],
    "gvk_gpa_bwd": [C.POINTER(GpaDesc), _P],
    "gvk_rows_broadcast": [_P, _P, _P, _I, _I, _I, _I, _I, _P],
    "gvk_rows_batch_sum": [_P, _P, _P, _I, _I, _I, _I, _I, _I, _P],
    "gvk_small_linear_fwd": [_P, _P, _P, _P, _I, _I, _I, _P],
    "gvk_small_linear_bwd": [_P, _P, _P, _P, _P, _P, _I, _I, _I, _I, _P],
    "gvk_vpt_repack_fwd": [_P, _P, _P, _I, _I, _I, _I, _I, _I, _P],
    "gvk_vpt_repack_bwd": [_P, _P, _I, _I, _I, _I, _I, _I, _P],
    "gvk_cast_bf16_f32_strided": [_P, _P, _I, _I, _I, _P],
    "gvk_lora_merge_f32": [_P, _P, _P, _P, _P, _P, _I, _I, _F, _P],
    "gvk_layernorm_fwd_proj": [_P, _P, _P, _P, _P, _P, _I, _I, _F, C.POINTER(RowProjDesc), _P],
    "gvk_layernorm_bwd_dy16": [C.POINTER(LnBwdDy16Desc), _P],
    "gvk_layernorm_bwd_proj": [_P, _P, _P, _P, _P, _P, _P, _P, _I, _I, C.POINTER(RowProjDesc), _P],
    "gvk_layernorm_bwd_up": [_P, _P, _P, _P, _P, _P, _P, _P, _P, _P, _I, _I, _I, _I, _P],
    "gvk_ssf_fold_weight": [_P, _P, _P, _P, _I, _I, _I, _P],
    "gvk_ssf_fold_vec": [_P, _P, _P, _P, _I, _P],
    "gvk_ssf_colgrad": [C.POINTER(SsfColgradDesc), _P],
    "gvk_ssf_ln_grad": [_P, _P, _P, _P, _P, _P, _I, _P],
    "gvk_ssf_head_grad": [_P, _P, _P, _P, _P, _P, _P, _P, _P, _I, _I, _I, _I, _I, _I, _P],
    "gvk_dvpt_fwd": [C.POINTER(DvptDesc), _P],
    "gvk_dvpt_bwd": [C.POINTER(DvptDesc), _P],
    "gvk_scale_dev": [_P, _P, C.c_int64, _P],
    "gvk_evp_highpass": [_P, _P, _P, _P, _I, _I, _I, _I, _P],
    "gvk_pad2d_f32": [_P, _I, _I, _I, _I, _P, _I, _I, _I, _P],
    "gvk_add2d_f32": [_P, _I, _P, _I, _P, _I, _I, _I, _P],
    "gvk_gelu_fwd_f32": [_P, _P, C.c_int64, _P],
    "gvk_gelu_bwd_f32": [_P, _P, _P, C.c_int64, _P],
    "gvk_rows_patch": [_P, _P, _P, _I, _I, _I, _I, _I, _I, _P],
    "gvk_rows_gather": [_P, _P, _I, _I, _I, _I, _I, _P],
    "gvk_sumsq": [_P, C.c_int64, _P, _P, _P],
    "gvk_adam_step": [C.POINTER(AdamDesc), _P],
    "gvk_loss_fwd_bwd": [C.POINTER(LossDesc), _P],
    "gvk_dropout_rows": [C.POINTER(DropoutDesc), _P],
    "gvk_volume_minmax": [_P, _P, _I, _L, _P],
    "gvk_rescale_intensity": [_P, _P, _P, _P, _I, _L, _F, _F, _P],
    "gvk_spatial_transform": [_P, _P, _P, _P, _P, _I, _I, _I, _I, _P],
    "gvk_eval_rows": [_P, _P, _P, _P, _P, _I, _I, _P],
    "gvk_ovr_auc_counts": [_P, _P, _P, _I, _I, _P],
    "gvk_memset_async": [_P, _I, C.c_size_t, _P],
    "gvk_seed_advance": [_P, C.c_uint64, _P],
    "gvk_scale_f32": [_P, _F, C.c_long, _P],
    "gvk_head_fwd": [C.POINTER(HeadDesc), _P],
    "gvk_head_bwd": [C.POINTER(HeadDesc), _P],
}
NO_STREAM = {"gvk_last_error": (C.c_char_p, []), "gvk_device_check": (C.c_int, []), "gvk_abi_version": (C.c_int, []),
             "gvk_attention_bwd_ws_bytes": (C.c_size_t, [C.c_int, C.c_int, C.c_int]),
             "gvk_attention_bwd_status_offset": (C.c_size_t, [C.c_size_t]),
             "gvk_gpa_gate_param_count": (C.c_int, [C.c_int, C.c_int]), "gvk_gemm_stat_parts": (C.c_int, [C.c_int]), "gvk_minmax_partials": (C.c_int, []),
             "gvk_param_grads_scratch": (C.c_int64, [C.POINTER(PgradOuter), C.c_int, C.POINTER(ReduceJob), C.c_int, C.c_int, C.c_int]),
             "gvk_plan_begin": (C.c_int, []), "gvk_plan_end": (C.c_int, []), "gvk_plan_abort": (C.c_int, []),
             "gvk_plan_size": (C.c_int, [C.c_int]), "gvk_plan_replay": (C.c_int, [C.c_int]), "gvk_plan_free": (C.c_int, [C.c_int]),
             "gvk_plan_event_record": (C.c_int, [_P]), "gvk_plan_event_wait": (C.c_int, [_P, C.c_int]),
             "gvk_plan_event_record_fenced": (C.c_int, [_P]), "gvk_plan_event_stream_wait": (C.c_int, [C.c_int, C.c_int, _P]),
             "gvk_plan_set_timing": (C.c_int, [C.c_int]),
             "gvk_plan_event_elapsed": (C.c_int, [C.c_int, C.c_int, C.c_int, C.POINTER(C.c_float)])}
STRUCTS = {"gvk_gemm_desc": GemmDesc, "gvk_skinny_down_desc": SkinnyDownDesc, "gvk_skinny_up_desc": SkinnyUpDesc,
           "gvk_outer_desc": OuterDesc, "gvk_window_attn_desc": WindowAttnDesc, "gvk_gpa_desc": GpaDesc, "gvk_head_desc": HeadDesc, "gvk_reduce_job": ReduceJob, "gvk_pgrad_outer": PgradOuter, "gvk_rowproj_desc": RowProjDesc, "gvk_adam_desc": AdamDesc, "gvk_loss_desc": LossDesc, "gvk_dropout_desc": DropoutDesc, "gvk_ssf_colgrad_desc": SsfColgradDesc, "gvk_dvpt_desc": DvptDesc}

DIAG_SIGNATURES = {}
DIAG_NO_STREAM = {"gvk_plan_nop_stream": (C.c_int, [_P]), "gvk_plan_nop_clear": (C.c_int, [])}

_lib = None


class GavikoHipError(RuntimeError):
    pass


def load() -> C.CDLL:
    global _lib
    if _lib is not None:
        return _lib
    if not os.path.exists(LIB_PATH):
        raise GavikoHipError(
            f"{LIB_PATH} not found: build it with `python -m gaviko_amd.build` (hipcc, gfx950). "
            "gaviko_amd has no CPU or eager fallback.")
    lib = C.CDLL(LIB_PATH)
    for name, (res, args) in NO_STREAM.items():
        fn = getattr(lib, name)
        fn.restype, fn.argtypes = res, args
    for name, args in SIGNATURES.items():
        fn = getattr(lib, name)
        fn.restype, fn.argtypes = C.c_int, args
    if DIAG:
        for name, (res, args) in DIAG_NO_STREAM.items():
            fn = getattr(lib, name)
            fn.restype, fn.argtypes = res, args
        for name, args in DIAG_SIGNATURES.items():
            fn = getattr(lib, name)
            fn.restype, fn.argtypes = C.c_int, args
    if lib.gvk_abi_version() != ABI_VERSION:
        raise GavikoHipError(f"{LIB_PATH} has ABI version {lib.gvk_abi_version()}, these bindings describe {ABI_VERSION}: rebuild with "
                             "`python -m gaviko_amd.build`")
    _lib = lib
    return lib


def check(rc: int, what: str) -> None:
    if rc != 0:
        raise GavikoHipError(f"{what} failed (rc={rc}): {load().gvk_last_error().decode()}")


_device_ok = False


def require_device() -> None:
    global _device_ok
    if _device_ok:
        return
    if not torch.cuda.is_available():
        raise GavikoHipError("no HIP device visible: gaviko_amd runs on MI355X (gfx950) only and has no CPU fallback")
    rc = load().gvk_device_check()
    if rc != 950:
        raise GavikoHipError(f"gvk_device_check: {load().gvk_last_error().decode()}")
    _device_ok = True


def stream_ptr() -> int:
    return torch.cuda.current_stream().cuda_stream


def ptr(t) -> int:
    return 0 if t is None else t.data_ptr()
```

gaviko_amd/ops.py:

```python
from __future__ import annotations

import ctypes as C

import torch

from . import lib as L
from .lib import (EPI_BIAS_GELU_BF16, EPI_BIAS_RELU_BF16, EPI_BIAS_RES_F32, EPI_BIAS_RES_F32_BF16, EPI_GELU_BWD_BF16,
                  EPI_PATCH_F32, EPI_RELU_BWD_BF16, EPI_STORE_BF16, EPI_STORE_F32)

ROW_PAD = 128


def pad_rows(m: int) -> int:
    return (m + ROW_PAD - 1) // ROW_PAD * ROW_PAD


def act_zeros(m: int, c: int, dtype, device) -> torch.Tensor:
    return torch.zeros((pad_rows(m), c), dtype=dtype, device=device)


def _chk(t, dtype, what, min_elems=0):
    if t is None:
        return
    if not t.is_cuda:
# ... 422 lines not shown
def skinny_up(**kw):
    d = _desc(L.SkinnyUpDesc, "skinny_up", **kw)
    L.check(L.load().gvk_skinny_up(C.byref(d), L.stream_ptr()), "gvk_skinny_up")


def outer_reduce(**kw):
    d = _desc(L.OuterDesc, "outer_reduce", **kw)
    L.check(L.load().gvk_outer_reduce(C.byref(d), L.stream_ptr()), "gvk_outer_reduce")


OUTER_MAX_ROWS = 10240


def outer_scratch_elems(Lat, C_):
    return 128 * (Lat + 1) * C_


def _reduce_jobs(jobs, what):
    arr = (L.ReduceJob * max(1, len(jobs)))()
    for k, job in enumerate(jobs):
        a, b, out, acc = job[:4]
        a2 = job[4] if len(job) > 4 else None
        for t, n in ((a, "a"), (b, "b"), (out, "out"), (a2, "a2")):
            _chk(t, torch.float32, f"{what} {n}")
        M, J = a.shape[0], a.numel() // a.shape[0]
        Lb = 0 if b is None else b.numel() // b.shape[0]
        if b is not None and b.shape[0] != M:
            raise L.GavikoHipError(f"{what}: a and b must have the same number of rows")
        if out.numel() < (J * Lb if b is not None else J):
            raise L.GavikoHipError(f"{what}: out too small")
        if a2 is not None and (b is not None or a2.numel() // a2.shape[0] != J):
            raise L.GavikoHipError(f"{what}: a2 goes with column sums of the same width only")
        arr[k] = L.ReduceJob(L.ptr(a), L.ptr(b), L.ptr(out), L.ptr(a2), M, J, Lb, int(bool(acc)), 0 if a2 is None else a2.shape[0])
    return arr


def param_grads_supported(Lat, C_):
    return C_ % 4 == 0 and 0 < Lat <= 28 and Lat % 4 == 0


PGRAD_TICKETS = 256


def param_grads(outer, small, scratch, tickets, C_, Lat, seed_ptr=None):
    arr = (L.PgradOuter * max(1, len(outer)))()
    fields = [f for f, _ in L.PgradOuter._fields_]
    for k, o in enumerate(outer):
        bad = set(o) - set(fields)
        if bad:
            raise L.GavikoHipError(f"param_grads: unknown field(s) {sorted(bad)}")
        vals = {}
        for f, ct in L.PgradOuter._fields_:
            v = o.get(f)
            if ct is C.c_void_p:
                _chk(v, torch.float32, f"param_grads outer[{k}].{f}")
                vals[f] = L.ptr(v)
            elif ct is C.c_float:
                vals[f] = float(v or 0.0)
            else:
                vals[f] = int(v or 0)
        M, M2, Cj = vals["M"], vals["M2"], vals["C"] or C_
        for f, n in (("narrow", M * Lat), ("wide", M * Cj), ("narrow2", M2 * Lat), ("wide2", M2 * Cj), ("mean", M), ("rstd", M), ("colsum", Cj),
                     ("out", Lat * Cj), ("aff_w", Lat * Cj), ("aff_gamma", Cj), ("aff_beta", Cj), ("aff_dgamma", Cj), ("aff_dbeta", Cj), ("aff_dbias", Lat)):
            if o.get(f) is not None and o[f].numel() < n:
                raise L.GavikoHipError(f"param_grads outer[{k}].{f}: needs >= {n} elements, has {o[f].numel()}")
        arr[k] = L.PgradOuter(**vals)
    jobs = _reduce_jobs(small, "param_grads small")
    _chk(scratch, torch.float32, "param_grads scratch")
    if tickets is None or tickets.dtype != torch.int32 or not tickets.is_cuda:
        raise L.GavikoHipError("param_grads: tickets must be an int32 tensor on the HIP device (zero at allocation)")
    L.check(L.load().gvk_param_grads(arr, len(outer), jobs, len(small), L.ptr(scratch), scratch.numel(), L.ptr(tickets), tickets.numel(),
                                     L.ptr(seed_ptr), C_, Lat, L.stream_ptr()), "gvk_param_grads")


def param_grads_scratch_elems(Lat, col_tiles, small_outputs):
    slabs = min(240 + sum(col_tiles), 64 * sum(col_tiles))
    return slabs * (Lat + 2) * 64 + sum(((o + 63) // 64) * 32 * 64 for o in small_outputs)


def small_wgrad(a, b, out, scratch, M, J, Lb, accumulate=False):
    for t, n in ((a, "a"), (b, "b"), (out, "out"), (scratch, "scratch")):
        _chk(t, torch.float32, "small_wgrad " + n)
    if scratch.numel() < 64 * J * Lb or a.numel() < M * J or b.numel() < M * Lb or out.numel() < J * Lb:
        raise L.GavikoHipError("small_wgrad: buffer too small")
    L.check(L.load().gvk_small_wgrad(L.ptr(a), L.ptr(b), L.ptr(out), L.ptr(scratch), M, J, Lb, int(accumulate), L.stream_ptr()), "gvk_small_wgrad")


def colsum(x, out, scratch, M, C_, accumulate=False):
    for t, n in ((x, "x"), (out, "out"), (scratch, "scratch")):
        _chk(t, torch.float32, "colsum " + n)
    if scratch.numel() < 64 * C_ or x.numel() < M * C_ or out.numel() < C_:
        raise L.GavikoHipError("colsum: buffer too small")
    L.check(L.load().gvk_colsum(L.ptr(x), L.ptr(out), L.ptr(scratch), M, C_, int(accumulate), L.stream_ptr()), "gvk_colsum")


def window_attn_fwd(**kw):
    d = _desc(L.WindowAttnDesc, "window_attn", **kw)
    L.check(L.load().gvk_window_attn_fwd(C.byref(d), L.stream_ptr()), "gvk_window_attn_fwd")


def window_attn_bwd(**kw):
    d = _desc(L.WindowAttnDesc, "window_attn", **kw)
    L.check(L.load().gvk_window_attn_bwd(C.byref(d), L.stream_ptr()), "gvk_window_attn_bwd")


def gpa_fwd(**kw):
    d = _desc(L.GpaDesc, "gpa", **kw)
    L.check(L.load().gvk_gpa_fwd(C.byref(d), L.stream_ptr()), "gvk_gpa_fwd")


def gpa_bwd(**kw):
    d = _desc(L.GpaDesc, "gpa", **kw)
    L.check(L.load().gvk_gpa_bwd(C.byref(d), L.stream_ptr()), "gvk_gpa_bwd")


def gpa_gate_param_count(Lat, P):
    return L.load().gvk_gpa_gate_param_count(Lat, P)


def rows_broadcast(out, src, add, B, T, row_off, R, C_):
    _chk(out, torch.float32, "rows_broadcast out", B * T * C_)
    _chk(src, torch.float32, "rows_broadcast src", R * C_)
    _chk(add, torch.float32, "rows_broadcast add", R * C_)
    L.check(L.load().gvk_rows_broadcast(L.ptr(out), L.ptr(src), L.ptr(add), B, T, row_off, R, C_, L.stream_ptr()), "gvk_rows_broadcast")


def rows_batch_sum(dg, out, out2, B, T, row_off, R, C_, accumulate=False):
    _chk(dg, torch.float32, "rows_batch_sum dg", B * T * C_)
    _chk(out, torch.float32, "rows_batch_sum out", R * C_)
    _chk(out2, torch.float32, "rows_batch_sum out2", R * C_)
    L.check(L.load().gvk_rows_batch_sum(L.ptr(dg), L.ptr(out), L.ptr(out2), B, T, row_off, R, C_, int(accumulate), L.stream_ptr()),
            "gvk_rows_batch_sum")


def head_fwd(**kw):
    d = _desc(L.HeadDesc, "head", **kw)
    L.check(L.load().gvk_head_fwd(C.byref(d), L.stream_ptr()), "gvk_head_fwd")


def head_bwd(**kw):
    d = _desc(L.HeadDesc, "head", **kw)
    L.check(L.load().gvk_head_bwd(C.byref(d), L.stream_ptr()), "gvk_head_bwd")


def attention_bwd_workspace(B, T, H, device):
    n = int(L.load().gvk_attention_bwd_ws_bytes(B, T, H))
    return torch.zeros((n + 3) // 4, dtype=torch.int32, device=device)


def attention_bwd_timeouts(ws) -> int:
    return int(ws[int(L.load().gvk_attention_bwd_status_offset(ws.numel() * 4)) // 4].item())


def attention_bwd(qkv, out, dout, lse, delta, dqkv, B, T, H, scale, drop_p=0.0, seed=0, seed_ptr=None, q_prescaled=False, ws=None, need_rows=None):
    inner = H * 64
    if qkv.dtype == torch.float32:
        for t, n, k in ((qkv, "qkv", 3), (out, "out", 1), (dout, "dout", 1), (dqkv, "dqkv", 3)):
            _chk(t, torch.float32, "attn_bwd " + n, B * T * k * inner)
        _chk(lse, torch.float32, "attn_bwd lse", B * H * T)
        _chk(delta, torch.float32, "attn_bwd delta", B * H * T)
        L.check(L.load().gvk_attention_bwd_f32_dropout(L.ptr(qkv), L.ptr(out), L.ptr(dout), L.ptr(lse), L.ptr(delta), L.ptr(dqkv), B, T, H,
                                                       3 * inner, inner, scale, float(drop_p), int(seed), L.ptr(seed_ptr) if drop_p > 0 else None,
                                                       L.stream_ptr()), "gvk_attention_bwd_f32")
        return
    _chk(qkv, torch.bfloat16, "attn_bwd qkv", pad_rows(B * T) * 3 * inner)
    _chk(out, torch.bfloat16, "attn_bwd out", pad_rows(B * T) * inner)
    _chk(dout, torch.bfloat16, "attn_bwd dout", pad_rows(B * T) * inner)
    _chk(dqkv, torch.bfloat16, "attn_bwd dqkv", B * T * 3 * inner)
    _chk(lse, torch.float32, "attn_bwd lse", B * H * T)
    _chk(delta, torch.float32, "attn_bwd delta", B * H * T)
    if not q_prescaled:
        qkv = _prescaled_copy(qkv, B * T, H, scale)
    if drop_p > 0:
        L.check(L.load().gvk_attention_bwd_bf16_dropout(L.ptr(qkv), L.ptr(out), L.ptr(dout), L.ptr(lse), L.ptr(delta), L.ptr(dqkv), B, T, H,
                                                        3 * inner, inner, scale, float(drop_p), int(seed), L.ptr(seed_ptr), L.stream_ptr()),
                "gvk_attention_bwd_bf16_dropout")
        return
    if need_rows is not None:
        L.check(L.load().gvk_attention_bwd_bf16_rows(L.ptr(qkv), L.ptr(out), L.ptr(dout), L.ptr(lse), L.ptr(delta), L.ptr(dqkv), B, T, H,
                                                     3 * inner, inner, scale, int(need_rows), L.stream_ptr()), "gvk_attention_bwd_bf16_rows")
        return
    if ws is not None:
        _chk(ws, torch.int32, "attn_bwd ws", (int(L.load().gvk_attention_bwd_ws_bytes(B, T, H)) + 3) // 4)
        L.check(L.load().gvk_attention_bwd_bf16_fused(L.ptr(qkv), L.ptr(out), L.ptr(dout), L.ptr(lse), L.ptr(delta), L.ptr(dqkv), L.ptr(ws),
                                                      ws.numel() * 4, B, T, H, 3 * inner, inner, scale, L.stream_ptr()), "gvk_attention_bwd_bf16_fused")
        return
    L.check(L.load().gvk_attention_bwd_bf16(L.ptr(qkv), L.ptr(out), L.ptr(dout), L.ptr(lse), L.ptr(delta), L.ptr(dqkv), B, T, H,
                                            3 * inner, inner, scale, L.stream_ptr()), "gvk_attention_bwd_bf16")


def small_linear_fwd(x, w, b, out, R, K, C_):
    for t, n in ((x, "x"), (w, "w"), (b, "b"), (out, "out")):
        _chk(t, torch.float32, "small_linear " + n)
    if x.numel() < R * K or w.numel() < C_ * K or out.numel() < R * C_:
        raise L.GavikoHipError("small_linear_fwd: buffer too small")
    L.check(L.load().gvk_small_linear_fwd(L.ptr(x), L.ptr(w), L.ptr(b), L.ptr(out), R, K, C_, L.stream_ptr()), "gvk_small_linear_fwd")


def small_linear_bwd(x, w, dout, dw, db, dx, R, K, C_, accumulate=False):
    for t, n in ((x, "x"), (w, "w"), (dout, "dout"), (dw, "dw"), (db, "db"), (dx, "dx")):
        _chk(t, torch.float32, "small_linear_bwd " + n)
    L.check(L.load().gvk_small_linear_bwd(L.ptr(x), L.ptr(w), L.ptr(dout), L.ptr(dw), L.ptr(db), L.ptr(dx), R, K, C_, int(accumulate),
                                          L.stream_ptr()), "gvk_small_linear_bwd")


def vpt_repack_fwd(inp, prompt, out, B, Tin, Tout, P, skip, C_):
    _chk(inp, torch.float32, "vpt_repack in", B * Tin * C_)
    _chk(prompt, torch.float32, "vpt_repack prompt", P * C_)
    _chk(out, torch.float32, "vpt_repack out", B * Tout * C_)
    L.check(L.load().gvk_vpt_repack_fwd(L.ptr(inp), L.ptr(prompt), L.ptr(out), B, Tin, Tout, P, skip, C_, L.stream_ptr()), "gvk_vpt_repack_fwd")


def vpt_repack_bwd(dout, din, B, Tin, Tout, P, skip, C_):
    _chk(dout, torch.float32, "vpt_repack_bwd dout", B * Tout * C_)
    _chk(din, torch.float32, "vpt_repack_bwd din", B * Tin * C_)
    L.check(L.load().gvk_vpt_repack_bwd(L.ptr(dout), L.ptr(din), B, Tin, Tout, P, skip, C_, L.stream_ptr()), "gvk_vpt_repack_bwd")


def cast_bf16_f32_strided(inp, out, M, C_, ld_in, col0=0):
    if inp.dtype == torch.float32:
        _chk(inp, torch.float32, "copy_strided in", M * ld_in)
        _chk(out, torch.float32, "copy_strided out", M * C_)
        L.check(L.load().gvk_copy_f32_strided(inp.data_ptr() + 4 * col0, L.ptr(out), M, C_, ld_in, L.stream_ptr()), "gvk_copy_f32_strided")
        return
    _chk(inp, torch.bfloat16, "cast_bf16_f32 in", M * ld_in)
    _chk(out, torch.float32, "cast_bf16_f32 out", M * C_)
    L.check(L.load().gvk_cast_bf16_f32_strided(inp.data_ptr() + 2 * col0, L.ptr(out), M, C_, ld_in, L.stream_ptr()), "gvk_cast_bf16_f32_strided")


def lora_merge(w, a_q, b_q, a_v, b_v, out, C_, r, s):
    for t, n in ((w, "w"), (a_q, "a_q"), (b_q, "b_q"), (a_v, "a_v"), (b_v, "b_v"), (out, "out")):
        _chk(t, torch.float32, "lora_merge " + n)
    if w.numel() != 3 * C_ * C_ or out.numel() < 3 * C_ * C_ or a_q.numel() != r * C_ or b_q.numel() != C_ * r:
        raise L.GavikoHipError("lora_merge: shape mismatch")
    L.check(L.load().gvk_lora_merge_f32(L.ptr(w), L.ptr(a_q), L.ptr(b_q), L.ptr(a_v), L.ptr(b_v), L.ptr(out), C_, r, float(s), L.stream_ptr()),
            "gvk_lora_merge_f32")


def reduce_batch(jobs, scratch):
    arr = (L.ReduceJob * len(jobs))()
    total = 0
    for k, job in enumerate(jobs):
        a, b, out, acc = job[:4]
        a2 = job[4] if len(job) > 4 else None
        _chk(a2, torch.float32, "reduce_batch a2")
        _chk(a, torch.float32, "reduce_batch a")
        _chk(b, torch.float32, "reduce_batch b")
        _chk(out, torch.float32, "reduce_batch out")
        M, J = a.shape[0], a.numel() // a.shape[0]
        Lb = 0 if b is None else b.numel() // b.shape[0]
        if b is not None and b.shape[0] != M:
            raise L.GavikoHipError("reduce_batch: a and b must have the same number of rows")
        if out.numel() < (J * Lb if b is not None else J):
            raise L.GavikoHipError("reduce_batch: out too small")
        total += J * Lb if b is not None else J
        if a2 is not None and (b is not None or a2.numel() // a2.shape[0] != J):
            raise L.GavikoHipError("reduce_batch: a2 goes with column sums of the same width only")
        arr[k] = L.ReduceJob(L.ptr(a), L.ptr(b), L.ptr(out), L.ptr(a2), M, J, Lb, int(bool(acc)), 0 if a2 is None else a2.shape[0])
    _chk(scratch, torch.float32, "reduce_batch scratch", 32 * total)
    L.check(L.load().gvk_reduce_batch(arr, len(jobs), L.ptr(scratch), L.stream_ptr()), "gvk_reduce_batch")


def ln_lowrank_affine(Q, S, W, gamma, beta, dW, dgamma, dbeta, dbias, Lat, C_, accumulate=False):
    for t, n in ((Q, "Q"), (S, "S"), (W, "W"), (gamma, "gamma"), (beta, "beta"), (dW, "dW"), (dgamma, "dgamma"), (dbeta, "dbeta"), (dbias, "dbias")):
        _chk(t, torch.float32, "ln_lowrank_affine " + n)
    if Q.numel() < Lat * C_ or W.numel() < Lat * C_ or dW.numel() < Lat * C_ or S.numel() < Lat:
        raise L.GavikoHipError("ln_lowrank_affine: buffer too small")
    L.check(L.load().gvk_ln_lowrank_affine(L.ptr(Q), L.ptr(S), L.ptr(W), L.ptr(gamma), L.ptr(beta), L.ptr(dW), L.ptr(dgamma), L.ptr(dbeta),
                                           L.ptr(dbias), Lat, C_, int(bool(accumulate)), L.stream_ptr()), "gvk_ln_lowrank_affine")


def ssf_fold_weight(w, s, out, out_t=None):
    _chk(w, torch.float32, "ssf_fold_weight w")
    N = w.shape[0]
    K = w.numel() // N
    _chk(s, torch.float32, "ssf_fold_weight s", N)
    if out.dtype not in (torch.bfloat16, torch.float32) or (out_t is not None and out_t.dtype != out.dtype):
        raise L.GavikoHipError("ssf_fold_weight: outputs must be bf16 or fp32 (both the same)")
    _chk(out, out.dtype, "ssf_fold_weight out", N * K)
    _chk(out_t, out.dtype, "ssf_fold_weight out_t", N * K)
    L.check(L.load().gvk_ssf_fold_weight(L.ptr(w), L.ptr(s), L.ptr(out), L.ptr(out_t), N, K, int(out.dtype == torch.float32), L.stream_ptr()),
            "gvk_ssf_fold_weight")


def ssf_fold_vec(a, s, t, out):
    n = s.numel()
    for x, nm in ((a, "a"), (s, "s"), (t, "t"), (out, "out")):
        _chk(x, torch.float32, "ssf_fold_vec " + nm, n)
    L.check(L.load().gvk_ssf_fold_vec(L.ptr(a), L.ptr(s), L.ptr(t), L.ptr(out), n, L.stream_ptr()), "gvk_ssf_fold_vec")


def ssf_colgrad(dy, y0, s, t, ds, dt, scratch, M, N, *, y1=None, pos=None, ld_dy=None, ld_y=None, rows_in=0, rows_out=0, row_off=0,
                y0_cols=0, y0_mul=1.0, y_mul=1.0):
    for x, nm in ((s, "s"), (t, "t"), (ds, "ds"), (dt, "dt")):
        _chk(x, torch.float32, "ssf_colgrad " + nm, N)
    _chk(scratch, torch.float32, "ssf_colgrad scratch", 64 * 2 * N)
    _chk(y1, torch.float32, "ssf_colgrad y1")
    _chk(pos, torch.float32, "ssf_colgrad pos")
    for x, nm in ((dy, "dy"), (y0, "y0")):
        if x.dtype not in (torch.bfloat16, torch.float32) or not x.is_cuda or not x.is_contiguous():
            raise L.GavikoHipError(f"ssf_colgrad {nm}: expected a contiguous bf16 / fp32 device tensor")
    d = L.SsfColgradDesc(dy=L.ptr(dy), y0=L.ptr(y0), y1=L.ptr(y1), pos=L.ptr(pos), s=L.ptr(s), t=L.ptr(t), ds=L.ptr(ds), dt=L.ptr(dt),
                         scratch=L.ptr(scratch), M=M, N=N, ld_dy=N if ld_dy is None else ld_dy, ld_y=N if ld_y is None else ld_y,
                         dy_f32=int(dy.dtype == torch.float32), y0_f32=int(y0.dtype == torch.float32), rows_in=rows_in, rows_out=rows_out,
                         row_off=row_off, y0_cols=int(y0_cols), y0_mul=float(y0_mul), y_mul=float(y_mul))
    L.check(L.load().gvk_ssf_colgrad(C.byref(d), L.stream_ptr()), "gvk_ssf_colgrad")


def ssf_ln_grad(dgamma_eff, dbeta_eff, gamma, beta, ds, dt):
    n = gamma.numel()
    for x, nm in ((dgamma_eff, "dgamma'"), (dbeta_eff, "dbeta'"), (gamma, "gamma"), (beta, "beta"), (ds, "ds"), (dt, "dt")):
        _chk(x, torch.float32, "ssf_ln_grad " + nm, n)
    L.check(L.load().gvk_ssf_ln_grad(L.ptr(dgamma_eff), L.ptr(dbeta_eff), L.ptr(gamma), L.ptr(beta), L.ptr(ds), L.ptr(dt), n, L.stream_ptr()),
            "gvk_ssf_ln_grad")


def ssf_head_grad(g, mean, rstd, wh, dlogits, gamma, beta, ds, dt, B, T, C_, K, r0, R):
    for x, nm in ((g, "g"), (mean, "mean"), (rstd, "rstd"), (wh, "wh"), (dlogits, "dlogits"), (gamma, "gamma"), (beta, "beta"), (ds, "ds"), (dt, "dt")):
        _chk(x, torch.float32, "ssf_head_grad " + nm)
    L.check(L.load().gvk_ssf_head_grad(L.ptr(g), L.ptr(mean), L.ptr(rstd), L.ptr(wh), L.ptr(dlogits), L.ptr(gamma), L.ptr(beta), L.ptr(ds),
                                       L.ptr(dt), B, T, C_, K, r0, R, L.stream_ptr()), "gvk_ssf_head_grad")


def dvpt_fwd(**kw):
    d = _desc(L.DvptDesc, "dvpt_fwd", **kw)
    L.check(L.load().gvk_dvpt_fwd(C.byref(d), L.stream_ptr()), "gvk_dvpt_fwd")


def dvpt_bwd(**kw):
    d = _desc(L.DvptDesc, "dvpt_bwd", **kw)
    L.check(L.load().gvk_dvpt_bwd(C.byref(d), L.stream_ptr()), "gvk_dvpt_bwd")


def scale_dev_(t: torch.Tensor, alpha: torch.Tensor) -> None:
    _chk(t, torch.float32, "scale_dev_ x")
    _chk(alpha, torch.float32, "scale_dev_ alpha", 1)
    L.check(L.load().gvk_scale_dev(L.ptr(t), L.ptr(alpha), t.numel(), L.stream_ptr()), "gvk_scale_dev")


def evp_highpass(img, hp, depth_mask, out):
    _chk(img, torch.float32, "evp_highpass img")
# ... 150 lines not shown
```

include/gaviko_hip.h:

```cpp
#ifndef GAVIKO_HIP_H
#define GAVIKO_HIP_H
#include <stddef.h>
#include <stdint.h>
#ifdef __cplusplus
extern "C" {
#endif

const char* gvk_last_error(void);
int gvk_device_check(void);
int gvk_abi_version(void);

int gvk_plan_begin(void);
int gvk_plan_end(void);
int gvk_plan_abort(void);
int gvk_plan_size(int plan);
int gvk_plan_replay(int plan);
int gvk_plan_free(int plan);
int gvk_plan_event_record(void* stream);
int gvk_plan_event_wait(void* stream, int event);
int gvk_plan_event_record_fenced(void* stream);
int gvk_plan_event_stream_wait(int plan, int event, void* stream);
int gvk_plan_set_timing(int on);
int gvk_plan_event_elapsed(int plan, int e0, int e1, float* ms);
int gvk_memset_async(void* ptr, int value, size_t bytes, void* stream);
int gvk_seed_advance(void* seed_u64, uint64_t inc, void* stream);
int gvk_scale_f32(float* x, float alpha, long n, void* stream);

enum gvk_epilogue {
  GVK_EPI_STORE_BF16 = 0,
  GVK_EPI_BIAS_RES_F32 = 1,
  GVK_EPI_BIAS_GELU_BF16 = 2,
  GVK_EPI_PATCH_F32 = 3,
  GVK_EPI_GELU_BWD_BF16 = 4,
  GVK_EPI_STORE_F32 = 5,
  GVK_EPI_BIAS_RES_F32_BF16 = 6,
  GVK_EPI_BIAS_RELU_BF16 = 7,
  GVK_EPI_RELU_BWD_BF16 = 8
};

typedef struct gvk_gemm_desc {
  const void* a;
  const void* w;
  void* out0;
  void* out1;
  const float* bias;
  const float* res;
  const void* aux;
  const float* pos;
  const void* seed_ptr;
  int32_t M, N, K;
  int32_t lda, ldw, ldo, ldres, ldaux;
  int32_t epilogue;
  int32_t rows_in, rows_out, row_off;
  int32_t tile;
  float drop_p;
  uint64_t seed;
  int32_t scale_cols;
  float col_scale;
  const float* ln_mean; const float* ln_rstd; const float* ln_c1;
  float* stat_part;
  const float* stat_pivot;
  int32_t m_panels, m_stride;
  void* splitk_ws; uint64_t splitk_ws_bytes;
  int32_t ksplit;
  int32_t aux_is_grad;
} gvk_gemm_desc;
int gvk_gemm_nt_bf16(const gvk_gemm_desc* d, void* stream);
int gvk_gemm_stat_parts(int N);

int gvk_gemm_nt_f32(const gvk_gemm_desc* d, void* stream);
int gvk_attention_fwd_f32(const float* qkv, float* out, float* lse, int B, int T, int H, int ld_qkv, int ld_out, float scale,
                          void* stream);
int gvk_attention_bwd_f32(const float* qkv, const float* out, const float* dout, const float* lse, float* delta, float* dqkv,
                          int B, int T, int H, int ld_qkv, int ld_out, float scale, void* stream);
int gvk_attention_fwd_f32_dropout(const float* qkv, float* out, float* lse, int B, int T, int H, int ld_qkv, int ld_out, float scale,
                                  float drop_p, uint64_t seed, const void* seed_ptr, void* stream);
int gvk_attention_bwd_f32_dropout(const float* qkv, const float* out, const float* dout, const float* lse, float* delta, float* dqkv,
                                  int B, int T, int H, int ld_qkv, int ld_out, float scale, float drop_p, uint64_t seed, const void* seed_ptr,
                                  void* stream);
int gvk_patchify_f32(const float* img, float* out, int B, int D, int H, int W, int pd, int ph, int pw, void* stream);
int gvk_transpose_f32(const float* in, float* out, int rows, int cols, void* stream);
int gvk_transpose_bf16(const void* in, void* out, int rows, int cols, void* stream);
int gvk_copy_f32_strided(const float* in, float* out, int M, int C, int ld_in, void* stream);
int gvk_copy_async(void* dst, const void* src, size_t bytes, void* stream);

int gvk_cast_f32_bf16(const float* in, void* out, int64_t n, void* stream);
int gvk_transpose_cast_f32_bf16(const float* in, void* out, int rows, int cols, void* stream);
int gvk_pack_split_bf16(const float* a, int ca, const float* b, void* dst, int ld_dst, int col0, int rows, int weight_side, void* stream);
int gvk_patchify_bf16(const float* img, void* out, int B, int D, int H, int W, int pd, int ph, int pw, void* stream);


int gvk_layernorm_fwd(const float* x, const float* gamma, const float* beta, void* y_bf16, float* y_f32,
                      float* mean, float* rstd, int M, int C, float eps, void* stream);
int gvk_layernorm_fwd_fix(float* x, const float* gamma, const float* beta, void* y_bf16, float* mean, float* rstd, int M, int C, float eps,
                          const float* enh, const float* lat, const float* wup, int T, int P, int L, void* stream);
int gvk_layernorm_bwd(const float* dy, const float* x, const float* mean, const float* rstd, const float* gamma,
                      const float* dres, float* dx, void* dx_bf16, int M, int C, void* stream);
int gvk_layernorm_bwd_rows(const float* dy, const float* x, const float* mean, const float* rstd, const float* gamma,
                           const float* dres, float* dx, void* dx_bf16, int groups, int rows_per_group, int group_stride, int C, void* stream);
int gvk_layernorm_bwd_affine(const float* dy, const float* x, const float* mean, const float* rstd, float* dgamma,
                             float* dbeta, float* scratch, int M, int C, int accumulate, void* stream);

typedef struct gvk_rowproj_desc {
  const float* w; const float* bias;
  float* y; float* z;
  void* y_split;
  int32_t L, w_layout, act;
  int32_t ld_split, col_split;
} gvk_rowproj_desc;
int gvk_layernorm_fwd_proj(const float* x, const float* gamma, const float* beta, void* y_bf16, float* mean, float* rstd,
                           int M, int C, float eps, const gvk_rowproj_desc* proj, void* stream);
int gvk_layernorm_bwd_proj(const float* dy, const float* x, const float* mean, const float* rstd, const float* gamma,
                           const float* dres, float* dx, void* dx_bf16, int M, int C, const gvk_rowproj_desc* proj, void* stream);
typedef struct gvk_ln_bwd_dy16_desc {
  const void* dy_bf16; const float* x; const float* mean; const float* rstd; const float* gamma; const float* dres;
  float* dx; void* dx_bf16;
  const gvk_rowproj_desc* proj;
  int32_t M, C, groups, rows_per_group, group_stride;
} gvk_ln_bwd_dy16_desc;
int gvk_layernorm_bwd_dy16(const gvk_ln_bwd_dy16_desc* d, void* stream);
int gvk_layernorm_bwd_up(const float* dy, const float* x, const float* mean, const float* rstd, const float* gamma, const float* dres,
                         float* dx, void* dx_bf16, const float* lat, const float* w, int w_layout, int M, int C, int L, void* stream);

int gvk_attention_fwd_bf16(const void* qkv, void* out, float* lse, int B, int T, int H, int ld_qkv, int ld_out, float scale,
                           void* stream);
int gvk_qkv_prescale_bf16(void* qkv, int rows, int H, int ld_qkv, float scale, void* stream);

int gvk_attention_bwd_bf16(const void* qkv, const void* out, const void* dout, const float* lse, float* delta, void* dqkv,
                           int B, int T, int H, int ld_qkv, int ld_out, float scale, void* stream);
size_t gvk_attention_bwd_ws_bytes(int B, int T, int H);
size_t gvk_attention_bwd_status_offset(size_t ws_bytes);
int gvk_attention_bwd_bf16_fused(const void* qkv, const void* out, const void* dout, const float* lse, float* delta, void* dqkv, void* ws,
                                 size_t ws_bytes, int B, int T, int H, int ld_qkv, int ld_out, float scale, void* stream);
int gvk_attention_colsum_bf16(const void* qkv, const float* lse, const float* w, int ld_w, float* out, int B, int T, int H, int ld_qkv,
                              int q0, int q1, void* stream);
int gvk_rollout_step(const float* r_in, const float* colsum, float* r_out, int B, int T, int H, void* stream);
int gvk_unpatchify_f32(const float* dcols, float* out, const float* x, const float* x0, int B, int D, int H, int W, int pd, int ph, int pw,
                       int nsum, float alpha, float beta, void* stream);
int gvk_patch_reduce_f32(const float* vol, float* out, int B, int D, int H, int W, int pd, int ph, int pw, int absval, void* stream);
int gvk_evp_highpass_sign(const float* img, const float* hp, const int32_t* depth_mask, const float* dout, float* out, int B, int D, int H, int W,
                          void* stream);
int gvk_evp_highpass_linear(const float* x, const float* op, const int32_t* depth_mask, float* out, int accumulate, int B, int D, int H, int W,
                            void* stream);
int gvk_attention_bwd_bf16_rows(const void* qkv, const void* out, const void* dout, const float* lse, float* delta, void* dqkv,
                                int B, int T, int H, int ld_qkv, int ld_out, float scale, int need_rows, void* stream);
int gvk_attention_fwd_bf16_dropout(const void* qkv, void* out, float* lse, int B, int T, int H, int ld_qkv, int ld_out, float scale,
                                   float drop_p, uint64_t seed, const void* seed_ptr, void* stream);
int gvk_attention_bwd_bf16_dropout(const void* qkv, const void* out, const void* dout, const float* lse, float* delta, void* dqkv,
                                   int B, int T, int H, int ld_qkv, int ld_out, float scale, float drop_p, uint64_t seed, const void* seed_ptr,
                                   void* stream);

typedef struct gvk_skinny_down_desc {
  const float* x; const float* w; const float* bias;
  const float* ln_gamma; const float* ln_beta; float* mean; float* rstd;
  float* z; float* y;
  const float* w2; float* y2;
  const uint64_t* seed_ptr;
  int32_t M, C, L, L2, act, w_layout;
  int32_t act_in;
  float eps, drop_p;
  uint64_t seed;
} gvk_skinny_down_desc;
int gvk_skinny_down(const gvk_skinny_down_desc* d, void* stream);

typedef struct gvk_skinny_up_desc {
  const float* lat; const float* w; const float* bias; const float* res; float* out; const float* lat_override;
  const uint64_t* seed_ptr;
  const float* ln_x; const float* ln_mean; const float* ln_rstd; const float* ln_gamma;
  void* out_bf16;
  const float* alpha_ptr;
  const float* gg_x;
  const float* w2; const float* bias2; float* z2; float* y2;
  const float* lat_b; const float* w_b;
  const float* nx_w; const float* nx_bias; const float* nx_ln_gamma; const float* nx_ln_beta; float* nx_mean; float* nx_rstd; float* nx_lat;
  const float* nx_w2; float* nx_y2;
  int32_t M, C, L, T, P, w_layout, accumulate;
  int32_t L2, act2, w2_layout, nx_L2;
  float drop_p, drop2_p, nx_eps;
  uint64_t seed, seed2;
} gvk_skinny_up_desc;
int gvk_skinny_up(const gvk_skinny_up_desc* d, void* stream);
int gvk_prompt_up_fix(const float* enh, const float* lat, const float* w, float* out, int B, int T, int P, int C, int L, void* stream);
int gvk_prompt_up_fix_stats(const float* enh, const float* lat, const float* w, float* out, void* out16, const float* part, int nparts,
                            const float* pivot, float* mean, float* rstd, int B, int T, int P, int C, int L, float eps, void* stream);

typedef struct gvk_outer_desc {
  const float* narrow; const float* wide; const float* lat_override;
  const float* mean; const float* rstd; const float* ln_gamma; const float* ln_beta;
  float* scratch; float* out; float* colsum;
  const uint64_t* seed_ptr;
  const float* narrow2; const float* wide2;
  int32_t M, C, L, T, P, transposed, accumulate;
  int32_t wide_act;
  int32_t M2;
  float drop_p;
  uint64_t seed;
} gvk_outer_desc;
int gvk_outer_reduce(const gvk_outer_desc* d, void* stream);
int gvk_ln_lowrank_affine(const float* Q, const float* S, const float* W, const float* gamma, const float* beta, float* dW, float* dgamma,
                          float* dbeta, float* dbias, int L, int C, int accumulate, void* stream);
int gvk_small_wgrad(const float* a, const float* b, float* out, float* scratch, int M, int J, int L, int accumulate, void* stream);
typedef struct gvk_reduce_job {
  const float* a; const float* b; float* out;
  const float* a2;
  int32_t M, J, L, accumulate, M2;
} gvk_reduce_job;
int gvk_reduce_batch(const gvk_reduce_job* jobs, int njobs, float* scratch, void* stream);
typedef struct gvk_pgrad_outer {
  const float* narrow; const float* wide; const float* narrow2; const float* wide2; const float* lat_override;
  const float* mean; const float* rstd;
  float* out; float* colsum;
  const float* aff_w; const float* aff_gamma; const float* aff_beta; float* aff_dgamma; float* aff_dbeta; float* aff_dbias;
  int32_t M, M2, T, P, transposed, accumulate;
  int32_t C;
  float drop_p;
  uint64_t seed;
} gvk_pgrad_outer;
int64_t gvk_param_grads_scratch(const gvk_pgrad_outer* outer, int n_outer, const gvk_reduce_job* small, int n_small, int C, int L);
int gvk_param_grads(const gvk_pgrad_outer* outer, int n_outer, const gvk_reduce_job* small, int n_small, float* scratch,
                    int64_t scratch_elems, int32_t* tickets, int n_tickets, const void* seed_ptr, int C, int L, void* stream);
int gvk_colsum(const float* x, float* out, float* scratch, int M, int C, int accumulate, void* stream);

typedef struct gvk_window_attn_desc {
  const float* qkv; float* ctx; float* lse;
  const float* dctx; float* delta; float* dqkv;
  const uint64_t* seed_ptr;
  int32_t B, D, H, W, kd, kh, kw, L;
  float scale, drop_p;
  uint64_t seed;
} gvk_window_attn_desc;
int gvk_window_attn_fwd(const gvk_window_attn_desc* d, void* stream);
int gvk_window_attn_bwd(const gvk_window_attn_desc* d, void* stream);

typedef struct gvk_gpa_desc {
  const float* xl; const float* ll;
  const float* ca0_g; const float* ca0_b; const float* ca1_w; const float* ca1_b; const float* ca3_w; const float* ca3_b;
  const float* gl0_g; const float* gl0_b; const float* gl1_w; const float* gl1_b;
  const float* wgq; const float* bgq; const float* wlq; const float* blq;
  float* imp; float* gw; float* enh;
  float* prm; float* qg; float* ql; float* cg; float* cl; float* lse_g; float* lse_l;
  const float* dcomb; const float* zx; const float* zl;
  float* dimp; float* dgw_part;
  float* dqg; float* dql; float* dcg; float* dcl; float* delta_g; float* delta_l; float* dprm;
  float* dcls; float* gate_partials; float* dzx; float* dzl;
  void* enh16;
  int32_t B, T, N, P, L, ld16, col16;
  float scale;
} gvk_gpa_desc;
int gvk_gpa_fwd(const gvk_gpa_desc* d, void* stream);
int gvk_gpa_bwd(const gvk_gpa_desc* d, void* stream);
int gvk_gpa_gate_param_count(int L, int P);

int gvk_rows_broadcast(float* out, const float* src, const float* add, int B, int T, int row_off, int R, int C, void* stream);
int gvk_rows_batch_sum(const float* dg, float* out, float* out2, int B, int T, int row_off, int R, int C, int accumulate, void* stream);
typedef struct gvk_head_desc {
  const float* g; const float* ln_gamma; const float* ln_beta; const float* wh; const float* bh;
  float* logits; float* pooled;
  const float* dlogits; float* dg; float* dwh; float* dbh;
  int32_t B, T, C, K, r0, R, accumulate;
} gvk_head_desc;
int gvk_head_fwd(const gvk_head_desc* d, void* stream);
int gvk_head_bwd(const gvk_head_desc* d, void* stream);

int gvk_small_linear_fwd(const float* x, const float* w, const float* b, float* out, int R, int K, int C, void* stream);
int gvk_small_linear_bwd(const float* x, const float* w, const float* dout, float* dw, float* db, float* dx, int R, int K, int C,
                         int accumulate, void* stream);
int gvk_vpt_repack_fwd(const float* in, const float* prompt, float* out, int B, int Tin, int Tout, int P, int skip, int C, void* stream);
int gvk_vpt_repack_bwd(const float* dout, float* din, int B, int Tin, int Tout, int P, int skip, int C, void* stream);
int gvk_lora_merge_f32(const float* w, const float* a_q, const float* b_q, const float* a_v, const float* b_v, float* out, int C, int r,
                       float s, void* stream);
int gvk_cast_bf16_f32_strided(const void* in, float* out, int M, int C, int ld_in, void* stream);

typedef struct gvk_ssf_colgrad_desc {
  const void* dy; const void* y0; const float* y1; const float* pos;
  const float* s; const float* t; float* ds; float* dt; float* scratch;
  int32_t M, N, ld_dy, ld_y, dy_f32, y0_f32, rows_in, rows_out, row_off;
  int32_t y0_cols;
  float y0_mul;
  float y_mul;
} gvk_ssf_colgrad_desc;
int gvk_ssf_fold_weight(const float* w, const float* s, void* out, void* out_t, int N, int K, int out_f32, void* stream);
int gvk_ssf_fold_vec(const float* a, const float* s, const float* t, float* out, int n, void* stream);
int gvk_ssf_colgrad(const gvk_ssf_colgrad_desc* d, void* stream);
int gvk_ssf_ln_grad(const float* dgamma_eff, const float* dbeta_eff, const float* gamma, const float* beta, float* ds, float* dt, int n,
                    void* stream);
int gvk_ssf_head_grad(const float* g, const float* mean, const float* rstd, const float* wh, const float* dlogits, const float* gamma,
                      const float* beta, float* ds, float* dt, int B, int T, int C, int K, int r0, int R, void* stream);

typedef struct gvk_dvpt_desc {
  const float* z; float* enh; float* lse;
  const float* dcomb; const float* gate; const float* bu; const float* colsum_dy;
  float* delta; float* dz; float* dgate;
  int32_t B, T, P, L, C;
  float scale;
} gvk_dvpt_desc;
int gvk_dvpt_fwd(const gvk_dvpt_desc* d, void* stream);
int gvk_dvpt_bwd(const gvk_dvpt_desc* d, void* stream);
int gvk_scale_dev(float* x, const float* alpha, int64_t n, void* stream);

int gvk_evp_highpass(const float* img, const float* hp, const int32_t* depth_mask, float* out, int B, int D, int H, int W, void* stream);
int gvk_pad2d_f32(const float* src, int ld_src, int rows, int cols, int transpose, float* dst, int ld_dst, int drows, int dcols, void* stream);
int gvk_add2d_f32(const float* a, int lda, const float* b, int ldb, float* out, int ldo, int rows, int cols, void* stream);
int gvk_gelu_fwd_f32(const float* x, float* y, int64_t n, void* stream);
// ... 45 lines not shown
```

Before: 770.3.

## Precompute attention-bwd augmented LSE/delta fragments in dQ kernel for dK/dV reuse

The dQ backward kernel now writes a per-query bf16x8 augmented fragment (scaled LSE, mask flag, delta) to a workspace. The dK/dV kernel stages these fragments into LDS with buffer loads and reads them directly, instead of loading fp32 lse/delta and rebuilding the fragment per sub-tile. This moves redundant per-tile conversion work out of the dK/dV inner loop. In exchange it adds a global write and read of the fragment workspace and a new API entry point that routes the engine through the presplit path.

```diff
diff --git a/gaviko_amd/csrc/attention_bwd.hip b/gaviko_amd/csrc/attention_bwd.hip
--- a/gaviko_amd/csrc/attention_bwd.hip
+++ b/gaviko_amd/csrc/attention_bwd.hip
@@ -3,14 +3,18 @@
 
 namespace gvk {
 
-template <int QT, bool DROP>
+__host__ __device__ constexpr int attn_aug_rows(int T) { return (T + 31) / 32 * 32; }
+constexpr int kAugRowBytes = 32;
+
+template <int QT, bool DROP, bool PRE>
 __global__ __launch_bounds__(256, 2) void attn_bwd_dkdv_kernel(const bf16* __restrict__ qkv, const bf16* __restrict__ d_o,
                                                             const float* __restrict__ lse, const float* __restrict__ delta,
-                                                            bf16* __restrict__ dqkv, int T, int H, int ld_qkv, int ld_o, float dk_scale,
-                                                            AttnDrop dr, int need_rows) {
+                                                            const bf16* __restrict__ aug, bf16* __restrict__ dqkv, int T, int H, int ld_qkv,
+                                                            int ld_o, float dk_scale, AttnDrop dr, int need_rows) {
   constexpr int NSB = QT / 32;
   constexpr int kTileQ = QT * 128;
-  constexpr int kBuf = 2 * kTileQ + 2 * 128 * 4;
+  constexpr int kAug = PRE ? QT * kAugRowBytes : 0;
+  constexpr int kBuf = 2 * kTileQ + (PRE ? kAug + (DROP ? 128 * 4 : 0) : 2 * 128 * 4);
   extern __shared__ __attribute__((aligned(16))) char smem[];
   int bh, kblk;
   xcd_group_block(blockIdx.x, (T + 127) / 128, gridDim.x / ((T + 127) / 128), bh, kblk);
@@ -37,7 +41,9 @@
   const int nB = (int)gridDim.x / (((T + 127) / 128) * H);
   const __amdgpu_buffer_rsrc_t rq = __builtin_amdgcn_make_buffer_rsrc((void*)qkv, 0, nB * T * ld_qkv * 2, 0x00020000);
   const __amdgpu_buffer_rsrc_t rd = __builtin_amdgcn_make_buffer_rsrc((void*)d_o, 0, nB * T * ld_o * 2, 0x00020000);
-  const __amdgpu_buffer_rsrc_t rl = __builtin_amdgcn_make_buffer_rsrc((void*)(wave < 2 ? lse : delta), 0, nB * H * T * 4, 0x00020000);
+  const __amdgpu_buffer_rsrc_t rl = __builtin_amdgcn_make_buffer_rsrc((void*)(wave < 2 && !PRE ? lse : delta), 0, nB * H * T * 4, 0x00020000);
+  const int Tq = attn_aug_rows(T);
+  [[maybe_unused]] const __amdgpu_buffer_rsrc_t ra = __builtin_amdgcn_make_buffer_rsrc((void*)aug, 0, nB * H * Tq * kAugRowBytes, 0x00020000);
   const int rsub = lane >> 3, slot = lane & 7;
   int voq[NSB], vod[NSB];
 #pragma unroll
@@ -49,11 +55,12 @@
   }
   const int lrow = (wave & 1) * 64 + lane;
   const int vol = ((b * H + head) * T + lrow) * 4;
-  auto stage = [&](int buf, int qt) {
+  [[maybe_unused]] const int voa = ((b * H + head) * Tq + wave * 32) * kAugRowBytes + lane * 16;
+  auto issue = [&](auto last_tag, int buf, int qt) {
+    constexpr bool last = decltype(last_tag)::value;
     char* sQ = smem + buf * kBuf;
     char* sD = sQ + kTileQ;
     char* sL = sD + kTileQ;
-    const bool last = qt == nqt - 1;
     const int soq = qt * QT * ld_qkv * 2, sod = qt * QT * ld_o * 2, sol = qt * QT * 4;
 #pragma unroll
     for (int r = 0; r < NSB; ++r) {
@@ -64,7 +71,19 @@
     }
     const int overl = last ? max(qt * QT + lrow - (T - 1), 0) : 0;
     const int vl = vol - overl * 4;
-    __builtin_amdgcn_raw_ptr_buffer_load_lds(rl, (GVK_LDS void*)(sL + (wave >> 1) * 512 + (wave & 1) * 256), 4, vl, sol, 0, 0);
+    if constexpr (PRE) {
+      const int soa = qt * QT * kAugRowBytes;
+      if (wave < NSB && qt * QT + wave * 32 < T)
+        __builtin_amdgcn_raw_ptr_buffer_load_lds(ra, (GVK_LDS void*)(sL + wave * 1024), 16, voa, soa, 0, 0);
+      if (DROP && wave < 2)
+        __builtin_amdgcn_raw_ptr_buffer_load_lds(rl, (GVK_LDS void*)(sL + kAug + wave * 256), 4, vl, sol, 0, 0);
+    } else {
+      __builtin_amdgcn_raw_ptr_buffer_load_lds(rl, (GVK_LDS void*)(sL + (wave >> 1) * 512 + (wave & 1) * 256), 4, vl, sol, 0, 0);
+    }
+  };
+  auto stage = [&](int buf, int qt) {
+    if (qt == nqt - 1) issue(std::true_type{}, buf, qt);
+    else issue(std::false_type{}, buf, qt);
   };
 
   f32x16 dkt[2], dvt[2];
@@ -82,13 +101,19 @@
       const char* sQ0 = smem + buf * kBuf;
       const char* sD0 = sQ0 + kTileQ;
       const float* sL0 = (const float*)(sD0 + kTileQ);
+      [[maybe_unused]] const float* sDl = PRE ? (const float*)(sD0 + kTileQ + kAug) : sL0 + 128;
       auto scores = [&](int sub, f32x16& s, f32x16& dp) {
-        const int qrow0 = qt * QT + sub * 32;
+        [[maybe_unused]] const int qrow0 = qt * QT + sub * 32;
         const char* sQ = sQ0 + sub * 32 * 128;
         const char* sD = sD0 + sub * 32 * 128;
-        const float l2 = sL0[sub * 32 + r31] * 1.44269504088896340736f;
-        const float dl = DROP ? 0.f : sL0[128 + sub * 32 + r31];
-        const bf16x8 qaug = aug_const(l2, qrow0 + r31 >= T, dl, hh);
+        bf16x8 qaug;
+        if constexpr (PRE) {
+          qaug = *(const bf16x8*)(sD0 + kTileQ + (sub * 32 + r31) * kAugRowBytes + hh * 16);
+        } else {
+          const float l2 = sL0[sub * 32 + r31] * 1.44269504088896340736f;
+          const float dl = DROP ? 0.f : sL0[128 + sub * 32 + r31];
+          qaug = aug_const(l2, qrow0 + r31 >= T, dl, hh);
+        }
         s = __builtin_amdgcn_mfma_f32_32x32x16_bf16(qaug, sel_s, f32x16{}, 0, 0, 0);
         if constexpr (DROP) dp = f32x16{};
         else dp = __builtin_amdgcn_mfma_f32_32x32x16_bf16(qaug, sel_d, f32x16{}, 0, 0, 0);
@@ -109,7 +134,7 @@
           if constexpr (DROP) {
             const unsigned int qq = (unsigned int)(qrow0 + (r & 3) + 8 * (r >> 2) + 4 * hh);
             const float mm = attn_drop_scale(akey, qq * (unsigned int)T + (unsigned int)key, dr.thresh, dr.inv_keep);
-            const float dlr = sL0[128 + sub * 32 + (r & 3) + 8 * (r >> 2) + 4 * hh];
+            const float dlr = sDl[sub * 32 + (r & 3) + 8 * (r >> 2) + 4 * hh];
             s[r] = pr * mm;
             dp[r] = pr * (dp[r] * mm - dlr);
           } else {
@@ -182,7 +207,7 @@
 
 template <int KB, bool DROP>
 __global__ __launch_bounds__(256, 2) void attn_bwd_dq_kernel(const bf16* __restrict__ qkv, const bf16* __restrict__ o_fwd, const bf16* __restrict__ d_o,
-                                                          const float* __restrict__ lse, float* __restrict__ delta,
+                                                          const float* __restrict__ lse, float* __restrict__ delta, bf16* __restrict__ aug,
                                                           bf16* __restrict__ dqkv, int T, int H, int ld_qkv, int ld_o, float scale,
                                                           AttnDrop dr, int need_rows) {
   constexpr int NKB = KB / 32;
@@ -210,13 +235,15 @@
   }
   del = half_sum(del);
   if (hh == 0 && q < T) delta[((size_t)b * H + head) * T + q] = del;
+  const float l2 = lse[((size_t)b * H + head) * T + qc] * 1.44269504088896340736f;
+  if (aug != nullptr && active)
+    *(bf16x8*)((char*)aug + (((size_t)b * H + head) * attn_aug_rows(T) + q) * kAugRowBytes + hh * 16) = aug_const(l2, q >= T, DROP ? 0.f : del, hh);
   if (q0 >= need_rows) return;
   [[maybe_unused]] unsigned int akey = 0u, qoff = 0u;
   if constexpr (DROP) {
     akey = attn_key(dr.seed + *dr.seed_ptr, b * H + head);
     qoff = (unsigned int)q * (unsigned int)T;
   }
-  const float l2 = lse[((size_t)b * H + head) * T + qc] * 1.44269504088896340736f;
   const bf16x8 qaug = aug_const(l2, true, DROP ? 0.f : del, hh);
   [[maybe_unused]] const bf16x8 sel_d = aug_sel_second(hh);
 
@@ -704,49 +731,78 @@
   store_rows_t(dvt, 1.0f, smem + wave * 8192 + 4096, dk_rows + inner, (size_t)ld_qkv, T - kw, lane);
 }
 
-template <int KB, bool DROP>
-static int launch_attn_bwd(const void* qkv, const void* out, const void* dout, const float* lse, float* delta, void* dqkv, int B, int T, int H,
-                           int ld_qkv, int ld_out, float scale, AttnDrop dr, hipStream_t s, int need_rows = 1 << 30) {
+template <int KB, bool DROP, bool PRE>
+static int launch_attn_bwd(const void* qkv, const void* out, const void* dout, const float* lse, float* delta, void* aug, void* dqkv, int B, int T,
+                           int H, int ld_qkv, int ld_out, float scale, AttnDrop dr, hipStream_t s, int need_rows) {
   const float dk_scale = 0.69314718055994530942f;
   const dim3 grid(((T + 127) / 128) * H * B);
-  constexpr unsigned lds_kv = 2 * (2 * KB * 128 + 2 * 128 * 4), lds_q = 2 * 2 * KB * 128;
+  constexpr unsigned lds_kv = 2 * (2 * KB * 128 + (PRE ? KB * kAugRowBytes + (DROP ? 128 * 4 : 0) : 2 * 128 * 4)), lds_q = 2 * 2 * KB * 128;
+  static_assert(2 * lds_kv <= 160 * 1024, "two dK/dV workgroups per CU");
   static bool attr = false;
   if (!attr) {
     hipError_t e = hipFuncSetAttribute(reinterpret_cast<const void*>(&attn_bwd_dq_kernel<KB, DROP>), hipFuncAttributeMaxDynamicSharedMemorySize, lds_q);
-    if (e == hipSuccess) e = hipFuncSetAttribute(reinterpret_cast<const void*>(&attn_bwd_dkdv_kernel<KB, DROP>), hipFuncAttributeMaxDynamicSharedMemorySize, lds_kv);
+    if (e == hipSuccess) e = hipFuncSetAttribute(reinterpret_cast<const void*>(&attn_bwd_dkdv_kernel<KB, DROP, PRE>), hipFuncAttributeMaxDynamicSharedMemorySize, lds_kv);
     if (e != hipSuccess) return set_error(-3, "hipFuncSetAttribute(attn_bwd): %s", hipGetErrorString(e));
     attr = true;
   }
-  GVK_LAUNCH((attn_bwd_dq_kernel<KB, DROP>), grid, dim3(256), lds_q, s, (const bf16*)qkv, (const bf16*)out, (const bf16*)dout, lse, delta, (bf16*)dqkv, T, H,
-             ld_qkv, ld_out, scale, dr, need_rows);
+  GVK_LAUNCH((attn_bwd_dq_kernel<KB, DROP>), grid, dim3(256), lds_q, s, (const bf16*)qkv, (const bf16*)out, (const bf16*)dout, lse, delta,
+             (bf16*)(PRE ? aug : nullptr), (bf16*)dqkv, T, H, ld_qkv, ld_out, scale, dr, need_rows);
   int rc = check_launch("attention_bwd/dq");
   if (rc) return rc;
-  GVK_LAUNCH((attn_bwd_dkdv_kernel<KB, DROP>), grid, dim3(256), lds_kv, s, (const bf16*)qkv, (const bf16*)dout, lse, (const float*)delta, (bf16*)dqkv, T, H,
-             ld_qkv, ld_out, dk_scale, dr, need_rows);
+  GVK_LAUNCH((attn_bwd_dkdv_kernel<KB, DROP, PRE>), grid, dim3(256), lds_kv, s, (const bf16*)qkv, (const bf16*)dout, lse, (const float*)delta,
+             (const bf16*)aug, (bf16*)dqkv, T, H, ld_qkv, ld_out, dk_scale, dr, need_rows);
   return check_launch("attention_bwd/dkdv");
 }
 
-}
-
-extern "C" int gvk_attention_bwd_bf16_dropout(const void* qkv, const void* out, const void* dout, const float* lse, float* delta, void* dqkv, int B,
-                                              int T, int H, int ld_qkv, int ld_out, float scale, float drop_p, uint64_t seed, const void* seed_ptr,
-                                              void* stream) {
-  using namespace gvk;
+static int attn_bwd_bf16(const void* qkv, const void* out, const void* dout, const float* lse, float* delta, void* aug, size_t aug_bytes,
+                         void* dqkv, int B, int T, int H, int ld_qkv, int ld_out, float scale, float drop_p, uint64_t seed, const void* seed_ptr,
+                         int need_rows, hipStream_t s) {
   GVK_REQUIRE(qkv && out && dout && lse && delta && dqkv, "gvk_attention_bwd_bf16: null pointer");
-  GVK_REQUIRE(B > 0 && T > 0 && H > 0, "gvk_attention_bwd_bf16: empty shape");
+  GVK_REQUIRE(B > 0 && T > 0 && H > 0 && need_rows > 0, "gvk_attention_bwd_bf16: empty shape");
   GVK_REQUIRE(ld_qkv >= 3 * H * 64 && ld_qkv % 8 == 0 && ld_out >= H * 64 && ld_out % 8 == 0,
               "gvk_attention_bwd_bf16: head dim is fixed at 64; ld_qkv=%d ld_out=%d inconsistent with H=%d", ld_qkv, ld_out, H);
   GVK_REQUIRE(drop_p >= 0.f && drop_p < 1.f && (drop_p == 0.f || seed_ptr != nullptr), "gvk_attention_bwd_bf16: drop_p in [0,1) and a seed word");
   GVK_REQUIRE(drop_p == 0.f || (int64_t)T * T < (int64_t)1 << 32, "gvk_attention_bwd_bf16: the dropout mask index (query*T + key) is 32-bit");
   GVK_REQUIRE((int64_t)B * T * ld_qkv * 2 < (int64_t)1 << 31, "gvk_attention_bwd_bf16: the qkv tensor must stay below 2 GiB (32-bit buffer offsets)");
+  if (aug != nullptr) {
+    const size_t need = (size_t)B * H * attn_aug_rows(T) * kAugRowBytes;
+    GVK_REQUIRE(aug_bytes >= need && ((uintptr_t)aug & 15) == 0, "gvk_attention_bwd_bf16_presplit: workspace of %zu bytes (16-byte aligned) needed, %zu given",
+                need, aug_bytes);
+    GVK_REQUIRE(need < ((size_t)1 << 31), "gvk_attention_bwd_bf16_presplit: the fragment workspace must stay below 2 GiB (32-bit buffer offsets)");
+  }
   const AttnDrop dr{seed, (const unsigned long long*)seed_ptr, drop_threshold_u32(drop_p), drop_p > 0.f ? 1.f / (1.f - drop_p) : 1.f};
-  hipStream_t s = (hipStream_t)stream;
   int kb = ((T + 95) / 96 * 96 < (T + 127) / 128 * 128) ? 96 : 128;
   if (getenv("GAVIKO_HIP_ATTN_KB") && (atoi(getenv("GAVIKO_HIP_ATTN_KB")) == 96 || atoi(getenv("GAVIKO_HIP_ATTN_KB")) == 128)) kb = atoi(getenv("GAVIKO_HIP_ATTN_KB"));
+#define GVK_ATTN_BWD(KB, DROP)                                                                                                                      \
+  (aug != nullptr ? launch_attn_bwd<KB, DROP, true>(qkv, out, dout, lse, delta, aug, dqkv, B, T, H, ld_qkv, ld_out, scale, dr, s, need_rows)    \
+                  : launch_attn_bwd<KB, DROP, false>(qkv, out, dout, lse, delta, aug, dqkv, B, T, H, ld_qkv, ld_out, scale, dr, s, need_rows))
   if (drop_p > 0.f)
-    return launch_attn_bwd<96, true>(qkv, out, dout, lse, delta, dqkv, B, T, H, ld_qkv, ld_out, scale, dr, s);
-  return kb == 96 ? launch_attn_bwd<96, false>(qkv, out, dout, lse, delta, dqkv, B, T, H, ld_qkv, ld_out, scale, dr, s)
-                  : launch_attn_bwd<128, false>(qkv, out, dout, lse, delta, dqkv, B, T, H, ld_qkv, ld_out, scale, dr, s);
+    return GVK_ATTN_BWD(96, true);
+  return kb == 96 ? GVK_ATTN_BWD(96, false) : GVK_ATTN_BWD(128, false);
+#undef GVK_ATTN_BWD
+}
+
+}
+
+extern "C" size_t gvk_attention_bwd_aug_bytes(int B, int T, int H) {
+  if (B <= 0 || T <= 0 || H <= 0) return 0;
+  return (size_t)B * H * gvk::attn_aug_rows(T) * gvk::kAugRowBytes;
+}
+
+extern "C" int gvk_attention_bwd_bf16_presplit(const void* qkv, const void* out, const void* dout, const float* lse, float* delta, void* aug,
+                                               size_t aug_bytes, void* dqkv, int B, int T, int H, int ld_qkv, int ld_out, float scale, float drop_p,
+                                               uint64_t seed, const void* seed_ptr, int need_rows, void* stream) {
+  using namespace gvk;
+  GVK_REQUIRE(aug != nullptr, "gvk_attention_bwd_bf16_presplit: null fragment workspace");
+  return attn_bwd_bf16(qkv, out, dout, lse, delta, aug, aug_bytes, dqkv, B, T, H, ld_qkv, ld_out, scale, drop_p, seed, seed_ptr,
+                       need_rows > 0 ? need_rows : 1 << 30, (hipStream_t)stream);
+}
+
+extern "C" int gvk_attention_bwd_bf16_dropout(const void* qkv, const void* out, const void* dout, const float* lse, float* delta, void* dqkv, int B,
+                                              int T, int H, int ld_qkv, int ld_out, float scale, float drop_p, uint64_t seed, const void* seed_ptr,
+                                              void* stream) {
+  return gvk::attn_bwd_bf16(qkv, out, dout, lse, delta, nullptr, 0, dqkv, B, T, H, ld_qkv, ld_out, scale, drop_p, seed, seed_ptr, 1 << 30,
+                            (hipStream_t)stream);
 }
 
 static constexpr int kFusedQT = 64;
@@ -811,16 +867,8 @@
 
 extern "C" int gvk_attention_bwd_bf16_rows(const void* qkv, const void* out, const void* dout, const float* lse, float* delta, void* dqkv, int B,
                                            int T, int H, int ld_qkv, int ld_out, float scale, int need_rows, void* stream) {
-  using namespace gvk;
-  GVK_REQUIRE(qkv && out && dout && lse && delta && dqkv, "gvk_attention_bwd_bf16_rows: null pointer");
-  GVK_REQUIRE(B > 0 && T > 0 && H > 0 && need_rows > 0, "gvk_attention_bwd_bf16_rows: empty shape");
-  GVK_REQUIRE(ld_qkv >= 3 * H * 64 && ld_qkv % 8 == 0 && ld_out >= H * 64 && ld_out % 8 == 0,
-              "gvk_attention_bwd_bf16_rows: head dim is fixed at 64; ld_qkv=%d ld_out=%d inconsistent with H=%d", ld_qkv, ld_out, H);
-  GVK_REQUIRE((int64_t)B * T * ld_qkv * 2 < (int64_t)1 << 31, "gvk_attention_bwd_bf16_rows: the qkv tensor must stay below 2 GiB (32-bit buffer offsets)");
-  const AttnDrop dr{0, nullptr, 0u, 1.f};
-  const int kb = ((T + 95) / 96 * 96 < (T + 127) / 128 * 128) ? 96 : 128;
-  return kb == 96 ? launch_attn_bwd<96, false>(qkv, out, dout, lse, delta, dqkv, B, T, H, ld_qkv, ld_out, scale, dr, (hipStream_t)stream, need_rows)
-                  : launch_attn_bwd<128, false>(qkv, out, dout, lse, delta, dqkv, B, T, H, ld_qkv, ld_out, scale, dr, (hipStream_t)stream, need_rows);
+  return gvk::attn_bwd_bf16(qkv, out, dout, lse, delta, nullptr, 0, dqkv, B, T, H, ld_qkv, ld_out, scale, 0.f, 0, nullptr, need_rows,
+                            (hipStream_t)stream);
 }
 
 extern "C" int gvk_attention_bwd_bf16(const void* qkv, const void* out, const void* dout, const float* lse, float* delta, void* dqkv, int B,
diff --git a/gaviko_amd/engine.py b/gaviko_amd/engine.py
--- a/gaviko_amd/engine.py
+++ b/gaviko_amd/engine.py
@@ -337,6 +337,7 @@
             ws["dctx"] = z(M, C, bf16)
             ws["dqkv"] = z(M, 3 * C, bf16)
             ws["delta"] = torch.zeros((B, self.heads, T), device=device)
+            ws["attn_aug"] = ops.attention_bwd_aug(B, max(self.Ts), self.heads, device)
             if self.kind == "gaviko":
                 Lt, P, BN = self.Lat, self.P, B * N
                 mk = lambda *s: torch.zeros(s, device=device)
@@ -1078,7 +1079,8 @@
         self._gemm(ws["dG16"], w[f"out{i}_t"], M, ws["dctx"], epilogue=ops.EPI_STORE_BF16)
         self._mark(f"b{i}:outd")
         ops.attention_bwd(ws["qkv"][i], ws["ctx"][i], ws["dctx"], ws["lse"][i], ws["delta"], ws["dqkv"], B, T, self.heads, 64 ** -0.5,
-                          drop_p=pd_, seed=SEED_LAYER + 8 * i, seed_ptr=ws["seed"], q_prescaled=True, need_rows=self.P if bot else None)
+                          drop_p=pd_, seed=SEED_LAYER + 8 * i, seed_ptr=ws["seed"], q_prescaled=True, need_rows=self.P if bot else None,
+                          aug=ws["attn_aug"])
         self._mark(f"b{i}:attnb")
         if self.kind == "melo" and i in self.lora_layers:
             self._melo_bwd(ws, gv, i, M)
diff --git a/gaviko_amd/lib.py b/gaviko_amd/lib.py
--- a/gaviko_amd/lib.py
+++ b/gaviko_amd/lib.py
@@ -124,6 +124,7 @@
     "gvk_attention_bwd_f32_dropout": [_P, _P, _P, _P, _P, _P, _I, _I, _I, _I, _I, _F, _F, C.c_uint64, _P, _P],
     "gvk_attention_fwd_bf16_dropout": [_P, _P, _P, _I, _I, _I, _I, _I, _F, _F, C.c_uint64, _P, _P],
     "gvk_attention_bwd_bf16_dropout": [_P, _P, _P, _P, _P, _P, _I, _I, _I, _I, _I, _F, _F, C.c_uint64, _P, _P],
+    "gvk_attention_bwd_bf16_presplit": [_P, _P, _P, _P, _P, _P, C.c_size_t, _P, _I, _I, _I, _I, _I, _F, _F, C.c_uint64, _P, _I, _P],
     "gvk_skinny_down": [C.POINTER(SkinnyDownDesc), _P],
     "gvk_skinny_up": [C.POINTER(SkinnyUpDesc), _P],
     "gvk_outer_reduce": [C.POINTER(OuterDesc), _P],
@@ -181,6 +182,7 @@
 NO_STREAM = {"gvk_last_error": (C.c_char_p, []), "gvk_device_check": (C.c_int, []), "gvk_abi_version": (C.c_int, []),
              "gvk_attention_bwd_ws_bytes": (C.c_size_t, [C.c_int, C.c_int, C.c_int]),
              "gvk_attention_bwd_status_offset": (C.c_size_t, [C.c_size_t]),
+             "gvk_attention_bwd_aug_bytes": (C.c_size_t, [C.c_int, C.c_int, C.c_int]),
              "gvk_gpa_gate_param_count": (C.c_int, [C.c_int, C.c_int]), "gvk_gemm_stat_parts": (C.c_int, [C.c_int]), "gvk_minmax_partials": (C.c_int, []),
              "gvk_param_grads_scratch": (C.c_int64, [C.POINTER(PgradOuter), C.c_int, C.POINTER(ReduceJob), C.c_int, C.c_int, C.c_int]),
              "gvk_plan_begin": (C.c_int, []), "gvk_plan_end": (C.c_int, []), "gvk_plan_abort": (C.c_int, []),
diff --git a/gaviko_amd/ops.py b/gaviko_amd/ops.py
--- a/gaviko_amd/ops.py
+++ b/gaviko_amd/ops.py
@@ -598,7 +598,12 @@
     return int(ws[int(L.load().gvk_attention_bwd_status_offset(ws.numel() * 4)) // 4].item())
 
 
-def attention_bwd(qkv, out, dout, lse, delta, dqkv, B, T, H, scale, drop_p=0.0, seed=0, seed_ptr=None, q_prescaled=False, ws=None, need_rows=None):
+def attention_bwd_aug(B, T, H, device):
+    return torch.empty(int(L.load().gvk_attention_bwd_aug_bytes(B, T, H)), dtype=torch.uint8, device=device)
+
+
+def attention_bwd(qkv, out, dout, lse, delta, dqkv, B, T, H, scale, drop_p=0.0, seed=0, seed_ptr=None, q_prescaled=False, ws=None, need_rows=None,
+                  aug=None):
     inner = H * 64
     if qkv.dtype == torch.float32:
         for t, n, k in ((qkv, "qkv", 3), (out, "out", 1), (dout, "dout", 1), (dqkv, "dqkv", 3)):
@@ -617,22 +622,18 @@
     _chk(delta, torch.float32, "attn_bwd delta", B * H * T)
     if not q_prescaled:
         qkv = _prescaled_copy(qkv, B * T, H, scale)
-    if drop_p > 0:
-        L.check(L.load().gvk_attention_bwd_bf16_dropout(L.ptr(qkv), L.ptr(out), L.ptr(dout), L.ptr(lse), L.ptr(delta), L.ptr(dqkv), B, T, H,
-                                                        3 * inner, inner, scale, float(drop_p), int(seed), L.ptr(seed_ptr), L.stream_ptr()),
-                "gvk_attention_bwd_bf16_dropout")
-        return
-    if need_rows is not None:
-        L.check(L.load().gvk_attention_bwd_bf16_rows(L.ptr(qkv), L.ptr(out), L.ptr(dout), L.ptr(lse), L.ptr(delta), L.ptr(dqkv), B, T, H,
-                                                     3 * inner, inner, scale, int(need_rows), L.stream_ptr()), "gvk_attention_bwd_bf16_rows")
-        return
-    if ws is not None:
+    if ws is not None and drop_p == 0 and need_rows is None:
         _chk(ws, torch.int32, "attn_bwd ws", (int(L.load().gvk_attention_bwd_ws_bytes(B, T, H)) + 3) // 4)
         L.check(L.load().gvk_attention_bwd_bf16_fused(L.ptr(qkv), L.ptr(out), L.ptr(dout), L.ptr(lse), L.ptr(delta), L.ptr(dqkv), L.ptr(ws),
                                                       ws.numel() * 4, B, T, H, 3 * inner, inner, scale, L.stream_ptr()), "gvk_attention_bwd_bf16_fused")
         return
-    L.check(L.load().gvk_attention_bwd_bf16(L.ptr(qkv), L.ptr(out), L.ptr(dout), L.ptr(lse), L.ptr(delta), L.ptr(dqkv), B, T, H,
-                                            3 * inner, inner, scale, L.stream_ptr()), "gvk_attention_bwd_bf16")
+    if aug is None:
+        aug = attention_bwd_aug(B, T, H, qkv.device)
+    _chk(aug, torch.uint8, "attn_bwd aug", int(L.load().gvk_attention_bwd_aug_bytes(B, T, H)))
+    L.check(L.load().gvk_attention_bwd_bf16_presplit(L.ptr(qkv), L.ptr(out), L.ptr(dout), L.ptr(lse), L.ptr(delta), L.ptr(aug), aug.numel(),
+                                                     L.ptr(dqkv), B, T, H, 3 * inner, inner, scale, float(drop_p), int(seed),
+                                                     L.ptr(seed_ptr) if drop_p > 0 else None, int(need_rows) if need_rows is not None and drop_p == 0 else 0,
+                                                     L.stream_ptr()), "gvk_attention_bwd_bf16_presplit")
 
 
 def small_linear_fwd(x, w, b, out, R, K, C_):
diff --git a/include/gaviko_hip.h b/include/gaviko_hip.h
--- a/include/gaviko_hip.h
+++ b/include/gaviko_hip.h
@@ -149,6 +149,10 @@
 int gvk_attention_bwd_bf16_dropout(const void* qkv, const void* out, const void* dout, const float* lse, float* delta, void* dqkv,
                                    int B, int T, int H, int ld_qkv, int ld_out, float scale, float drop_p, uint64_t seed, const void* seed_ptr,
                                    void* stream);
+size_t gvk_attention_bwd_aug_bytes(int B, int T, int H);
+int gvk_attention_bwd_bf16_presplit(const void* qkv, const void* out, const void* dout, const float* lse, float* delta, void* aug,
+                                    size_t aug_bytes, void* dqkv, int B, int T, int H, int ld_qkv, int ld_out, float scale, float drop_p,
+                                    uint64_t seed, const void* seed_ptr, int need_rows, void* stream);
 
 typedef struct gvk_skinny_down_desc {
   const float* x; const float* w; const float* bias;
```

After: 774.8 (median of 6 runs). About the same (+0.6%).
